# UbiquitousLearning/Mandheling-DSP-Training

Measured on AMD Instinct MI355X. Metric: training images/sec + int8 MFMA TOPS, VGG-11 batch 256, 1/2/4/8 MI355X, higher is better.
Workload: dtype int8; 1 GPU; VGG11 NITI int8 training step (fwd+relu+pool, loss grad, weight grad, input grad, SGD), 3x32x32; global_batch=256, per_gpu_batch=256, parallelism=single GPU, streams=one stream (weight gradient, then input gradient, per layer)

## Files before the change

include/niti_hip.h:

```cpp
#ifndef NITI_HIP_H
#define NITI_HIP_H

#include <stddef.h>
#include <stdint.h>

#ifdef __cplusplus
extern "C" {
#endif

enum niti_error_code {
    NITI_NO_ERROR = 0,
    NITI_OUT_OF_MEMORY = 1,
    NITI_NOT_SUPPORT = 2,
    NITI_COMPUTE_SIZE_ERROR = 3,
    NITI_NO_EXECUTION = 4,
    NITI_INVALID_VALUE = 5,
    NITI_INPUT_DATA_ERROR = 10,
    NITI_CALL_BACK_STOP = 11
};

enum niti_op_type {
    NITI_OP_CONV_INT8 = 700,
    NITI_OP_DECONV_INT8 = 701,
    NITI_OP_RELU_INT8 = 703,
// ... 44 lines not shown
    int kernel_x, kernel_y;
    int stride_x, stride_y;
    int dilate_x, dilate_y;
    int pad_x, pad_y;
    int has_pads;
    int pads[4];
    int pad_mode;
    int input_count, output_count;
    int group;
} niti_conv2d_common;

typedef struct niti_execution* niti_execution_t;

int niti_create_execution(int op_type, const niti_conv2d_common* common, niti_execution_t* out);

int niti_execution_resize(niti_execution_t e, const niti_tensor* inputs, int n_in, const niti_tensor* outputs,
                          int n_out);
int niti_execution_execute(niti_execution_t e, const niti_tensor* inputs, int n_in, const niti_tensor* outputs,
                           int n_out, void* stream);
int niti_execution_status(niti_execution_t e, void* stream);
void niti_destroy_execution(niti_execution_t e);
size_t niti_execution_workspace_bytes(niti_execution_t e);
int niti_tensor_convert(const niti_tensor* src, const niti_tensor* dst, void* stream);

#define NITI_MAX_WORDS 2048
typedef struct niti_geom {
    int n, c_in, h, w, c_out, kh, kw;
    int stride_h, stride_w, pad_t, pad_l, pad_b, pad_r, dilate_h, dilate_w;
    int oh, ow, cip, cop, np;
} niti_geom;

int niti_geom_finalize(niti_geom* g);

int niti_conv_workspace_bytes(const niti_geom* g, int op, size_t* bytes);
int niti_conv_plan_info(const niti_geom* g, int op, size_t ws_bytes, int info[4]);
int niti_conv_plan_set(const niti_geom* g, int op, const int plan[4]);
int niti_matmul_workspace_bytes(int m, int ldc, int k16, size_t* bytes);
int niti_conv_fwd_acc(const niti_geom* g, const int8_t* x_nhwc16, const int8_t* w_ohwi16, int32_t* acc,
                      uint32_t* amax, void* workspace, size_t workspace_bytes, void* stream);
int niti_conv_dgrad_acc(const niti_geom* g, const int8_t* dy_nhwc16, const int8_t* wt_ihwo16, int32_t* acc,
                        uint32_t* amax, void* workspace, size_t workspace_bytes, void* stream);
int niti_conv_fwd_phase1(const niti_geom* g, const int8_t* x_nhwc16, const int8_t* w_ohwi16, int32_t* acc,
                         uint32_t* amax, void* workspace, size_t workspace_bytes, void* stream);
int niti_conv_fwd_phase2(const niti_geom* g, const int8_t* x_nhwc16, const int8_t* w_ohwi16, const int32_t* acc,
                         const uint32_t* amax, const int8_t* exp_in, const int8_t* wscale, int8_t* exp_out, int relu,
                         const int8_t* relu_mask, int8_t* out_nhwc16, size_t workspace_bytes, void* stream);
int niti_conv_dgrad_phase1(const niti_geom* g, const int8_t* dy_nhwc16, const int8_t* wt_ihwo16, int32_t* acc,
                           uint32_t* amax, void* workspace, size_t workspace_bytes, void* stream);
int niti_conv_dgrad_phase2(const niti_geom* g, const int8_t* dy_nhwc16, const int8_t* wt_ihwo16, const int32_t* acc,
                           const uint32_t* amax, const int8_t* exp_in, const int8_t* wscale, int8_t* exp_out,
                           int relu, const int8_t* relu_mask, int8_t* out_nhwc16, size_t workspace_bytes,
                           void* stream);
#define NITI_ROWCONV_STATE_WORDS 1216
uint32_t* niti_rows_spec_slot(uint32_t* state, int dgrad);
int niti_conv_rows_ok(const niti_geom* g);
int niti_nhwc16_to_c32(const int8_t* in_nhwc16, int n, int hw, int cp, int c, int8_t* out_c32, void* stream);
int niti_weights_to_wf(const int8_t* w_ohwi16, int co, int ci, int cip, int transpose, int8_t* out_wf,
                       void* stream);
#define NITI_ROWS_X_NHWC16 0x100
int niti_conv_rows_nhwc_ok(const niti_geom* g, int flags);
int niti_conv_fwd_rows(const niti_geom* g, const int8_t* x_c32, const int8_t* wf, const int8_t* exp_in,
                       const int8_t* wscale, int8_t* exp_out, int relu, int8_t* out_nhwc16, int8_t* pool_out_nhwc16,
                       int8_t* next_c32, int mode, uint32_t* amax, uint32_t* state, uint32_t epoch, uint32_t* err,
                       void* stream);
int niti_conv_dgrad_rows(const niti_geom* g, const int8_t* dy_c32, const int8_t* wft, const int8_t* relu_mask,
                         const int8_t* pool_x, const int8_t* pool_y, int pool_relu, int8_t* dx_nhwc16, int8_t* dx_c32,
                         int8_t* dx_p16, const int8_t* exp_in, const int8_t* wscale, int8_t* exp_out, int mode,
                         uint32_t* amax, uint32_t* state, uint32_t epoch, uint32_t* err, void* stream);
int niti_conv_wgrad_acc(const niti_geom* g, const int8_t* x_nhwc16, const int8_t* dy_nhwc16, int32_t* acc,
                        uint32_t* amax, void* workspace, size_t workspace_bytes, void* stream);
int niti_nhwc16_to_p16(const int8_t* in_nhwc16, int64_t pixels, int cp, int8_t* out_p16, void* stream);
int niti_conv_wgrad_p16_workspace(const niti_geom* g, int splits, size_t* bytes);
void niti_diag_wgrad_stamps(void* buf);
void niti_diag_rowconv_stamps(void* buf);
void niti_diag_rowconv_barrier(uint32_t spin_limit, uint32_t expect_extra);
void niti_diag_rowconv_speculate(int mode);
void niti_diag_gemm_speculate(int bias);
unsigned long long niti_diag_gemm_fused_launches(void);
unsigned long long niti_diag_head_chain_launches(void);
void niti_diag_head_chain(int on);
void niti_diag_p16_jobs_cap(int cap);
int niti_conv_wgrad_p16_acc(const niti_geom* g, const int8_t* x_p16, const int8_t* dy_p16, int32_t* acc,
                            uint32_t* amax, void* workspace, size_t workspace_bytes, int splits, void* stream);
int niti_matmul_acc(int m, int o, int k16, const int8_t* B, int64_t ldb, const int8_t* A, int64_t lda,
                    int32_t* acc, int64_t ldc, uint32_t* amax, void* workspace, size_t workspace_bytes,
                    void* stream);
int niti_absmax_i32(const int32_t* acc, int64_t n, uint32_t* amax, void* stream);
int niti_requant_act(const int32_t* acc, int64_t rows, int ldc, const uint32_t* amax, const int8_t* exp_in,
                     const int8_t* wscale, int8_t* exp_out, int relu, const int8_t* relu_mask, int8_t* out_nhwc16,
                     void* stream);
typedef struct niti_requant_fused {
    const int8_t* exp_in;
    const int8_t* wscale;
    int8_t* exp_out;
    const int8_t* relu_mask;
    int8_t* out_nhwc16;
    int8_t* pool_out;
    const int8_t* pool_x;
    const int8_t* pool_y;
    int8_t* pool_dx;
    int8_t* pool_dx_c32;
    int8_t* out_p16;
    int8_t* pool3_out;
    int8_t* pool3_arg;
    int relu, pool_relu, pool_h, pool_w;
    int zero_cls, zc_h, zc_w;
    int pool3_h, pool3_w, pool3_oh, pool3_ow;
} niti_requant_fused;
int niti_requant_act_fused(const int32_t* acc, int64_t rows, int ldc, const uint32_t* amax,
                           const niti_requant_fused* f, void* stream);
int niti_requant_grad(const int32_t* acc, int64_t n, const uint32_t* amax, int rule, int8_t* g_out,
                      int8_t* w_update, void* stream);
int niti_sgd_update(const int32_t* acc, const uint32_t* amax, int rule, int co, int ci, int kk, int cip, int cop,
                    int8_t* w_ohwi16, int8_t* wt_ihwo16, int8_t* g_out, void* stream);
int niti_sgd_update_wf(const int32_t* acc, const uint32_t* amax, int rule, int co, int ci, int kk, int cip, int cop,
                       int8_t* w_ohwi16, int8_t* wt_ihwo16, int8_t* g_out, int8_t* wf, int8_t* wft, void* stream);
int niti_nhwc16_to_chwn16(const int8_t* in, int n, int hw, int cp, int np, int8_t* out, void* stream);
int niti_ohwi16_to_ihwo16(const int8_t* w, int co, int ci, int kk, int cip, int cop, int8_t* wt, void* stream);
int niti_nchw_to_nhwc16(const int8_t* x, int n, int c, int hw, int cp, int8_t* out, void* stream);
int niti_nchw_to_chwn16(const int8_t* x, int n, int c, int hw, int cp, int np, int8_t* out, void* stream);
int niti_nhwc16_to_nchw(const int8_t* x, int n, int c, int hw, int cp, int8_t* out, void* stream);
int niti_oihw_to_ohwi16(const int8_t* w, int co, int ci, int kk, int cip, int8_t* out, void* stream);
int niti_ohwi16_to_oihw(const int8_t* w, int co, int ci, int kk, int cip, int8_t* out, void* stream);
int niti_residual_add(const int8_t* a, const int8_t* ea, const int8_t* b, const int8_t* eb, int64_t n, int32_t* z,
                      int8_t* ez, uint32_t* amax, void* stream);
int niti_residual_requant(const int8_t* a, const int8_t* ea, const int8_t* b, const int8_t* eb, int64_t n,
                          const uint32_t* amax, int8_t* ez, int8_t* exp_out, int relu, int8_t* out, void* stream);
int niti_residual_requant_relu_grad(const int8_t* a, const int8_t* ea, const int8_t* b, const int8_t* eb, int64_t n,
                                    const uint32_t* amax, int8_t* ez, int8_t* exp_out, const int8_t* relu_mask,
                                    int8_t* out, void* stream);
int niti_sum_pool(const int8_t* x, int n, int hw, int cp, int32_t* acc, uint32_t* amax, void* stream);
int niti_sum_pool_grad(const int8_t* dy, int n, int hw, int cp, int8_t* dx, void* stream);
int niti_im2col(const niti_geom* g, const int8_t* x, int kp, int8_t* xcol, void* stream);
int niti_im2col_nchw(const niti_geom* g, const int8_t* x_nchw, int kp, int8_t* xcol, void* stream);
int niti_maxpool(const int8_t* x, int n, int h, int w, int cp, int k, int s, int p, int8_t* y, int oh, int ow,
                 void* stream);
int niti_maxpool_grad(const int8_t* x, const int8_t* y, const int8_t* dy, int n, int h, int w, int cp, int k,
                      int s, int p, int oh, int ow, int relu, int8_t* dx, void* stream);
int niti_maxpool_grad_ws(const int8_t* x, const int8_t* y, const int8_t* dy, int n, int h, int w, int cp, int k,
                         int s, int p, int oh, int ow, int relu, int8_t* workspace, int8_t* dx, void* stream);
int niti_maxpool_arg(const int8_t* x, int n, int h, int w, int cp, int k, int s, int p, int8_t* y, int oh, int ow,
                     int8_t* arg, void* stream);
int niti_maxpool_grad_arg(const int8_t* x, const int8_t* arg, const int8_t* dy, int n, int h, int w, int cp, int k,
                          int s, int p, int oh, int ow, int relu, const int8_t* pooled, int8_t* dx, void* stream);
int niti_relu_grad(const int8_t* x, const int8_t* dy, int64_t n, int8_t* out, void* stream);
int niti_loss_grad(const int8_t* logits, int batch, int classes, int ld, const int8_t* ascale,
                   const int32_t* labels, int8_t* out, void* stream);
typedef struct niti_eval_totals {
    uint64_t images, top1, topk;
    double loss_sum;
} niti_eval_totals;
int niti_head_metrics(const int8_t* logits, int batch, int classes, int ld, const int8_t* ascale,
                      const int32_t* labels, int topk, int32_t* pred ,
                      double* loss_per_image , niti_eval_totals* totals ,
                      void* workspace, size_t workspace_bytes, void* stream);
int niti_head_metrics_workspace(int batch, size_t* bytes);

int niti_image_stats(const uint8_t* images_nchw, int64_t n, uint64_t* stats, void* stream);
int niti_image_quantize(const uint8_t* images_nchw, int n, int c, int hw, const uint64_t* stats, int64_t count,
                        int8_t* out_nchw, int8_t* ascale, void* stream);
int niti_image_quantize_nhwc16(const uint8_t* images_nchw, int n, int c, int hw, int cp, const uint64_t* stats,
                               int64_t count, int8_t* out_nhwc16, int8_t* ascale, void* stream);

enum niti_arch { NITI_ARCH_LENET = 1, NITI_ARCH_VGG11 = 2, NITI_ARCH_VGG16 = 3, NITI_ARCH_RESNET18 = 4 };
typedef struct niti_model* niti_model_t;

// ... 73 lines not shown
```

mandheling-dsp-training_amd/csrc/niti_capi.hip:

```cpp
#include "../../include/niti_hip.h"
#include <memory>
#include <vector>

#include "niti_internal.hpp"
#include "niti_kernels.hpp"

struct niti_execution {
    niti::Execution* impl = nullptr;
    int op = 0;
    std::vector<void*> stage;
    std::vector<size_t> stage_bytes;
    uint32_t* err_host = nullptr;
    ~niti_execution() {
        delete impl;
        for (void* p : stage)
            if (p) (void)hipFree(p);
        if (err_host) (void)hipHostFree(err_host);
    }
};

namespace {
int code(hipError_t e) {
    if (e == hipSuccess) return NITI_NO_ERROR;
    if (e == hipErrorOutOfMemory) return NITI_OUT_OF_MEMORY;
// ... 367 lines not shown
                         void* ws, size_t ws_bytes, void* stream) {
    if (!g || !x || !w || !acc || !amax) return NITI_INVALID_VALUE;
    niti::ConvGeom r;
    if (!to_geom(g, &r)) return NITI_COMPUTE_SIZE_ERROR;
    return code(niti::conv_fwd_phase1(r, x, w, acc, amax, ws, ws ? ws_bytes : 0, S(stream)));
}

int niti_conv_fwd_phase2(const niti_geom* g, const int8_t* x, const int8_t* w, const int32_t* acc,
                         const uint32_t* amax, const int8_t* exp_in, const int8_t* wscale, int8_t* exp_out, int relu,
                         const int8_t* relu_mask, int8_t* out, size_t ws_bytes, void* stream) {
    if (!g || !x || !w || !acc || !amax || !out) return NITI_INVALID_VALUE;
    niti::ConvGeom r;
    if (!to_geom(g, &r)) return NITI_COMPUTE_SIZE_ERROR;
    return code(niti::conv_fwd_phase2(r, x, w, acc, amax, act_out(exp_in, wscale, exp_out, relu, relu_mask, out),
                                      ws_bytes, S(stream)));
}

int niti_conv_dgrad_phase1(const niti_geom* g, const int8_t* dy, const int8_t* wt, int32_t* acc, uint32_t* amax,
                           void* ws, size_t ws_bytes, void* stream) {
    if (!g || !dy || !wt || !acc || !amax) return NITI_INVALID_VALUE;
    niti::ConvGeom r;
    if (!to_geom(g, &r)) return NITI_COMPUTE_SIZE_ERROR;
    return code(niti::conv_dgrad_phase1(r, dy, wt, acc, amax, ws, ws ? ws_bytes : 0, S(stream)));
}

int niti_conv_dgrad_phase2(const niti_geom* g, const int8_t* dy, const int8_t* wt, const int32_t* acc,
                           const uint32_t* amax, const int8_t* exp_in, const int8_t* wscale, int8_t* exp_out, int relu,
                           const int8_t* relu_mask, int8_t* out, size_t ws_bytes, void* stream) {
    if (!g || !dy || !wt || !acc || !amax || !out) return NITI_INVALID_VALUE;
    niti::ConvGeom r;
    if (!to_geom(g, &r)) return NITI_COMPUTE_SIZE_ERROR;
    return code(niti::conv_dgrad_phase2(r, dy, wt, acc, amax, act_out(exp_in, wscale, exp_out, relu, relu_mask, out),
                                        ws_bytes, S(stream)));
}

int niti_conv_wgrad_acc(const niti_geom* g, const int8_t* x, const int8_t* dy, int32_t* acc, uint32_t* amax,
                        void* ws, size_t ws_bytes, void* stream) {
    if (!g) return NITI_INVALID_VALUE;
    niti::ConvGeom r;
    if (!to_geom(g, &r)) return NITI_COMPUTE_SIZE_ERROR;
    return code(niti::conv_wgrad_acc(r, x, dy, acc, amax, ws, ws_bytes, S(stream)));
}

int niti_nhwc16_to_p16(const int8_t* in, int64_t pixels, int cp, int8_t* out, void* stream) {
    if (!in || !out || pixels <= 0 || pixels % 16 || cp <= 0 || cp % 16) return NITI_INVALID_VALUE;
    return code(niti::nhwc16_to_p16(in, pixels, cp, out, S(stream)));
}

void niti_diag_wgrad_stamps(void* buf) { niti::wgrad_stamps_arm((unsigned long long*)buf); }
void niti_diag_rowconv_stamps(void* buf) { niti::rowconv_stamps_arm((unsigned long long*)buf); }
uint32_t* niti_rows_spec_slot(uint32_t* state, int dgrad) {
    return state ? niti::rowconv_spec_slot(state, dgrad != 0) : nullptr;
}

void niti_diag_rowconv_barrier(uint32_t spin_limit, uint32_t expect_extra) {
    niti::rowconv_barrier_diag(spin_limit, expect_extra);
}
void niti_diag_rowconv_speculate(int mode) { niti::rowconv_speculate(mode); }
void niti_diag_gemm_speculate(int bias) { niti::gemm_speculate_bias(bias); }
unsigned long long niti_diag_gemm_fused_launches(void) { return niti::gemm_fused_launches(); }
unsigned long long niti_diag_head_chain_launches(void) { return niti::head_chain_launches(); }
void niti_diag_head_chain(int on) { niti::head_chain_enable(on); }
void niti_diag_p16_jobs_cap(int cap) { niti::model_p16_jobs_cap(cap); }

int niti_conv_wgrad_p16_workspace(const niti_geom* g, int splits, size_t* bytes) {
    if (!g || !bytes) return NITI_INVALID_VALUE;
    niti::ConvGeom r;
    if (!to_geom(g, &r)) return NITI_COMPUTE_SIZE_ERROR;
    if (!niti::conv_wgrad_p16_ok(r)) return NITI_NOT_SUPPORT;
    *bytes = niti::conv_wgrad_p16_workspace(r, splits);
    return NITI_NO_ERROR;
}

int niti_conv_wgrad_p16_acc(const niti_geom* g, const int8_t* x, const int8_t* dy, int32_t* acc, uint32_t* amax,
                            void* ws, size_t ws_bytes, int splits, void* stream) {
    if (!g || !x || !dy || !acc) return NITI_INVALID_VALUE;
    niti::ConvGeom r;
    if (!to_geom(g, &r)) return NITI_COMPUTE_SIZE_ERROR;
    if (!niti::conv_wgrad_p16_ok(r)) return NITI_NOT_SUPPORT;
    if (splits <= 0) splits = niti::conv_wgrad_p16_splits(r);
    if (ws_bytes < niti::conv_wgrad_p16_workspace(r, splits) || (ws_bytes > 0 && !ws)) return NITI_INVALID_VALUE;
    return code(niti::conv_wgrad_p16(r, x, dy, acc, amax, ws, ws_bytes, splits, S(stream)));
}

int niti_matmul_acc(int m, int o, int k16, const int8_t* B, int64_t ldb, const int8_t* A, int64_t lda, int32_t* acc,
                    int64_t ldc, uint32_t* amax, void* ws, size_t ws_bytes, void* stream) {
    if (k16 % 16 || ldb % 16 || lda % 16 || ldc % 16 || ldc < o) return NITI_INVALID_VALUE;
    return code(niti::matmul_acc(m, o, k16, B, ldb, A, lda, acc, ldc, amax, ws, ws_bytes, S(stream)));
}

int niti_absmax_i32(const int32_t* acc, int64_t n, uint32_t* amax, void* stream) {
    return code(niti::absmax_i32(acc, n, amax, S(stream)));
}

int niti_requant_act(const int32_t* acc, int64_t rows, int ldc, const uint32_t* amax, const int8_t* exp_in,
                     const int8_t* wscale, int8_t* exp_out, int relu, const int8_t* relu_mask, int8_t* out,
                     void* stream) {
    niti::ActRequant r;
    r.acc = acc;
    r.rows = rows;
    r.ldc = ldc;
    r.amax = amax;
    r.exp_in = exp_in;
    r.wscale = wscale;
    r.exp_out = exp_out;
    r.relu = relu;
    r.relu_mask = relu_mask;
    r.out_nhwc16 = out;
    return code(niti::requant_act(r, S(stream)));
}

int niti_requant_act_fused(const int32_t* acc, int64_t rows, int ldc, const uint32_t* amax,
                           const niti_requant_fused* f, void* stream) {
    if (!f || rows < 0) return NITI_INVALID_VALUE;
    niti::ActRequant r;
    r.acc = acc;
    r.rows = rows;
    r.ldc = ldc;
    r.amax = amax;
    r.exp_in = f->exp_in;
    r.wscale = f->wscale;
    r.exp_out = f->exp_out;
    r.relu = f->relu;
    r.relu_mask = f->relu_mask;
    r.out_nhwc16 = f->out_nhwc16;
    r.pool.pool_out = f->pool_out;
    r.pool.x = f->pool_x;
    r.pool.y = f->pool_y;
    r.pool.dx = f->pool_dx;
    r.pool.relu = f->pool_relu;
    r.pool.H = f->pool_h;
    r.pool.W = f->pool_w;
    r.pool.dx_c32 = f->pool_dx_c32;
    r.out_p16 = f->out_p16;
    r.zero_cls = f->zero_cls;
    r.zc_h = f->zc_h;
    r.zc_w = f->zc_w;
    r.pool3.out = f->pool3_out;
    r.pool3.arg = f->pool3_arg;
    r.pool3.H = f->pool3_h;
    r.pool3.W = f->pool3_w;
    r.pool3.OH = f->pool3_oh;
    r.pool3.OW = f->pool3_ow;
    return code(niti::requant_act(r, S(stream)));
}

int niti_requant_grad(const int32_t* acc, int64_t n, const uint32_t* amax, int rule, int8_t* g_out, int8_t* w,
                      void* stream) {
    if (rule != 2 && rule != 3) return NITI_INVALID_VALUE;
    return code(niti::requant_grad(acc, n, amax, rule, g_out, w, S(stream)));
}

int niti_sgd_update(const int32_t* acc, const uint32_t* amax, int rule, int co, int ci, int kk, int cip, int cop,
                    int8_t* w, int8_t* wt, int8_t* g_out, void* stream) {
    if (rule != 2 && rule != 3) return NITI_INVALID_VALUE;
    return code(niti::sgd_update(acc, amax, rule, co, ci, kk, cip, cop, w, wt, g_out, S(stream)));
}
int niti_sgd_update_wf(const int32_t* acc, const uint32_t* amax, int rule, int co, int ci, int kk, int cip, int cop,
                       int8_t* w, int8_t* wt, int8_t* g_out, int8_t* wf, int8_t* wft, void* stream) {
    if (rule != 2 && rule != 3) return NITI_INVALID_VALUE;
    if ((wf || wft) && (kk != 9 || ci % 32 != 0 || co % 32 != 0)) return NITI_NOT_SUPPORT;
    niti::SgdJob j{acc, amax, rule, co, ci, kk, cip, cop, w, wt, g_out};
    j.wf = wf;
    j.wft = wft;
    return code(niti::sgd_update_many(&j, 1, S(stream)));
}
// ... 231 lines not shown
```

mandheling-dsp-training_amd/csrc/niti_kernels.hip:

```cpp
#include <stdlib.h>

#include <map>
#include <atomic>
#include <mutex>
#include <type_traits>
#include <vector>
#include <algorithm>
#include <stdio.h>

#include <hip/hip_ext.h>

#include "niti_device.hpp"
#include "niti_gridbar.hpp"
#include "niti_kernels.hpp"
#include "niti_sgd.hpp"
#include "niti_map.hpp"

namespace niti {


bool ConvGeom::finalize() {
    if (n <= 0 || c_in <= 0 || h <= 0 || w <= 0 || c_out <= 0 || kh <= 0 || kw <= 0) return false;
    if (sh <= 0 || sw <= 0 || dh <= 0 || dw <= 0) return false;
    const int keh = dh * (kh - 1) + 1, kew = dw * (kw - 1) + 1;
// ... 3670 lines not shown
        }
        if (live) {
            const v4i* base = (const v4i*)(J.slab + e);
            const int64_t st4 = J.slab_stride / 4;
            v4i s = {0, 0, 0, 0};
            for (int z0 = 0; z0 < J.splits; z0 += 8) {
                v4i v[8];
#pragma unroll
                for (int q = 0; q < 8; ++q)
                    v[q] = z0 + q < J.splits ? __builtin_nontemporal_load(base + (int64_t)(z0 + q) * st4) : v4i{0, 0, 0, 0};
#pragma unroll
                for (int q = 0; q < 8; ++q) s += v[q];
            }
            *(v4i*)(const_cast<int32_t*>(J.acc) + de) = s;
#pragma unroll
            for (int q = 0; q < 4; ++q) {
                const uint32_t u = uabs32(s[q]);
                m = m > u ? m : u;
            }
        }
    }
    if (cur >= 0) {
        const uint32_t w = wave_max(m);
        if ((threadIdx.x & 63) == 0) publish_max(const_cast<uint32_t*>(jobs.job[cur].amax), w);
    }
}

__global__ void sgd_update_kernel(SgdJobs jobs, int total) {
    __shared__ int8_t T[64][64 + 4];
    struct Tile {
        int j, ci0, co0, k;
    };
    auto locate = [&](int bb) {
        Tile t;
        int b = bb, j = 0;
        while (j + 1 < jobs.n && b >= jobs.start[j + 1]) ++j;
        const SgdJob& J = jobs.job[j];
        b -= jobs.start[j];
        const int tx = (J.cip + 63) / 64, ty = (J.cop + 63) / 64;
        const int k = b / (tx * ty), rem = b - k * tx * ty;
        t.j = j;
        t.ci0 = (rem % tx) * 64;
        t.co0 = (rem / tx) * 64;
        t.k = k;
        return t;
    };
    int bb = blockIdx.x;
    if (bb >= total) return;
    if (!NITI_SGD_PREFETCH) {
        int last_j = -1, bw = 0;
        for (; bb < total; bb += gridDim.x) {
            const Tile t = locate(bb);
            if (t.j != last_j) {
                bw = bitwidth_of(read_max(jobs.job[t.j].amax));
                last_j = t.j;
            }
            if (bb != (int)blockIdx.x) __syncthreads();
            sgd_tile(jobs.job[t.j], bw, t.ci0, t.co0, t.k, T);
        }
        return;
    }
    Tile cur = locate(bb);
    SgdTileIn cin, nin;
    sgd_tile_load(jobs.job[cur.j], cur.ci0, cur.co0, cur.k, cin);
    int last_j = -1, bw = 0;
    for (; bb < total; bb += gridDim.x) {
        const int nb = bb + gridDim.x;
        Tile nxt = cur;
        if (nb < total) {
            nxt = locate(nb);
            sgd_tile_load(jobs.job[nxt.j], nxt.ci0, nxt.co0, nxt.k, nin);
        }
        if (cur.j != last_j) {
            bw = bitwidth_of(read_max(jobs.job[cur.j].amax));
            last_j = cur.j;
        }
        if (bb != (int)blockIdx.x) __syncthreads();
        sgd_tile_finish(jobs.job[cur.j], bw, cur.ci0, cur.co0, cur.k, cin, T);
        cur = nxt;
        cin = nin;
    }
}

hipError_t sgd_update_many(const SgdJob* jobs, int n, hipStream_t st) {
    if (n <= 0) return hipSuccess;
    if (n > SGD_MAX_JOBS) return hipErrorInvalidValue;
    SgdJobs J{};
    J.n = n;
    int total = 0, chunks = 0;
    for (int i = 0; i < n; ++i) {
        J.job[i] = jobs[i];
        J.start[i] = total;
        J.cstart[i] = chunks;
        total += ((jobs[i].cip + 63) / 64) * ((jobs[i].cop + 63) / 64) * jobs[i].kk;
        if (jobs[i].slab != nullptr) {
            if (jobs[i].splits < 1 || jobs[i].slab_stride % 4 != 0 || jobs[i].slab_n % 4 != 0) return hipErrorInvalidValue;
            chunks += (int)((jobs[i].slab_n + 1023) / 1024);
        }
    }
    J.cstart[n] = chunks;
    if (chunks > 0) {
        const int cgrid = chunks < 2048 ? chunks : 2048;
        hipLaunchKernelGGL(sgd_combine_kernel, dim3(cgrid), dim3(256), 0, st, J);
    }
    const int grid = total < 1536 ? total : 1536;
    hipLaunchKernelGGL(sgd_update_kernel, dim3(grid), dim3(256), 0, st, J, total);
    return hipGetLastError();
}

hipError_t sgd_update(const int32_t* acc, const uint32_t* amax, int rule, int co, int ci, int kk, int cip, int cop,
                      int8_t* w, int8_t* wT, int8_t* g_out, hipStream_t st) {
    SgdJob j{acc, amax, rule, co, ci, kk, cip, cop, w, wT, g_out};
    return sgd_update_many(&j, 1, st);
}


__global__ void maxpool_kernel(const int8_t* __restrict__ x, int n, int h, int w, int cp, int k, int s, int p,
                               int8_t* __restrict__ y, int oh, int ow, int8_t* __restrict__ arg) {
    const uint32_t groups = cp / 16;
    const uint32_t total = (uint32_t)n * oh * ow * groups;
    const int kh = k < h ? k : h, kw = k < w ? k : w;
    for (uint32_t t = blockIdx.x * blockDim.x + threadIdx.x; t < total; t += gridDim.x * blockDim.x) {
        uint32_t r = t;
        const int gi = (int)(r % groups);
        r /= groups;
        const int ox = (int)(r % (uint32_t)ow);
        r /= (uint32_t)ow;
        const int oy = (int)(r % (uint32_t)oh);
        const int b = (int)(r / (uint32_t)oh);
        const int sx0 = ox * s - p, sy0 = oy * s - p;
        v16c m, a;
#pragma unroll
        for (int j = 0; j < 16; ++j) {
            m[j] = (signed char)-128;
            a[j] = (signed char)-1;
        }
        for (int yy = max(0, -sy0); yy < min(kh, h - sy0); ++yy)
            for (int xx = max(0, -sx0); xx < min(kw, w - sx0); ++xx) {
                const v16c v = *(const v16c*)(x + (((int64_t)b * h + sy0 + yy) * w + sx0 + xx) * cp + gi * 16);
                const signed char pos = (signed char)(yy * k + xx);
#pragma unroll
                for (int j = 0; j < 16; ++j) {
                    const bool take = a[j] < 0 || v[j] > m[j];
                    m[j] = take ? v[j] : m[j];
                    a[j] = take ? pos : a[j];
                }
            }
        *(v16c*)(y + (int64_t)t * 16) = m;
        if (arg != nullptr && (kh < k || kw < k)) {
#pragma unroll
            for (int j = 0; j < 16; ++j) a[j] = (signed char)-1;
            for (int yy = max(0, -sy0); yy < min(k, h - sy0); ++yy)
                for (int xx = max(0, -sx0); xx < min(k, w - sx0); ++xx) {
                    const v16c v = *(const v16c*)(x + (((int64_t)b * h + sy0 + yy) * w + sx0 + xx) * cp + gi * 16);
                    const signed char pos = (signed char)(yy * k + xx);
#pragma unroll
                    for (int j = 0; j < 16; ++j) a[j] = (a[j] < 0 && v[j] >= m[j]) ? pos : a[j];
                }
        }
        if (arg != nullptr) *(v16c*)(arg + (int64_t)t * 16) = a;
    }
}

hipError_t maxpool_nhwc16(const int8_t* x, int n, int h, int w, int cp, int k, int s, int p, int8_t* y, int oh, int ow,
                          hipStream_t st, int8_t* arg) {
    const int64_t total = (int64_t)n * oh * ow * (cp / 16);
// ... 641 lines not shown
```

mandheling-dsp-training_amd/csrc/niti_kernels.hpp:

```cpp
#pragma once

#include <hip/hip_runtime.h>
#include <stdint.h>
#include <stdlib.h>

#include "../../include/niti_hip.h"

namespace niti {

inline int round_up(int x, int m) { return (x + m - 1) / m * m; }

constexpr int MAX_SLOTS = 64;
constexpr int MAX_SLOT_STRIDE = 32;
constexpr int MAX_WORDS = MAX_SLOTS * MAX_SLOT_STRIDE;
constexpr size_t MAX_BYTES = MAX_WORDS * sizeof(uint32_t);

struct ConvGeom {
    int n, c_in, h, w;
    int c_out, kh, kw;
    int sh, sw, pt, pl, pb, pr, dh, dw;
    int oh, ow;
    int cip, cop, np;
    bool finalize();
};

enum GradRule { RULE_WGRAD_BW2 = 2, RULE_MATMUL_BW3 = 3 };

size_t conv_fwd_workspace(const ConvGeom& g);
size_t conv_dgrad_workspace(const ConvGeom& g);
size_t conv_wgrad_workspace(const ConvGeom& g);
size_t matmul_workspace(int M, int ldc, int k16);

enum PlanOp { PLAN_FWD = 0, PLAN_DGRAD = 1, PLAN_WGRAD = 2, PLAN_MATMUL = 3 };
struct PlanKey {
    int op, M, N, K;
    bool operator<(const PlanKey& o) const {
        if (op != o.op) return op < o.op;
        if (M != o.M) return M < o.M;
        if (N != o.N) return N < o.N;
        return K < o.K;
    }
};
struct PlanChoice {
    int bm = 128, bn = 128, splits = 1, strat = 0;
};
constexpr int PLAN_TAPS_TILE = 32;
constexpr int PLAN_P16_TILE = 16;
bool plan_override_lookup(const PlanKey& k, PlanChoice* c);
bool conv_wgrad_taps_ok(const ConvGeom& g);
PlanKey conv_plan_key(int op, const ConvGeom& g);
PlanChoice conv_plan_query(int op, const ConvGeom& g, bool recompute_ok, size_t ws_bytes);
int conv_plan_k_step(int op, const ConvGeom& g);
void plan_override_set(const PlanKey& k, const PlanChoice& c);
void plan_override_clear(const PlanKey& k);
void plan_override_clear_all();
unsigned plan_override_epoch();
PlanChoice plan_query(const PlanKey& k, int k_step, bool recompute_ok, size_t ws_bytes);
size_t plan_slab_bytes(int M, int N, int splits);
struct PlanChoice;
size_t conv_wgrad_slab_bytes(const ConvGeom& g, const PlanChoice& c);
hipError_t conv_fwd_acc(const ConvGeom& g, const int8_t* x_nhwc16, const int8_t* w_ohwi16, int32_t* acc,
                        uint32_t* amax, void* ws, size_t ws_bytes, hipStream_t st);
hipError_t conv_dgrad_acc(const ConvGeom& g, const int8_t* dy_nhwc16, const int8_t* wt_ihwo16, int32_t* acc,
                          uint32_t* amax, void* ws, size_t ws_bytes, hipStream_t st);
void probe_span_arm(unsigned long long* slot);
constexpr int SPAN_MAX_BLOCKS = 4096;
void probe_events_arm(hipEvent_t begin, hipEvent_t end);
struct SgdJob;
hipError_t conv_wgrad_acc(const ConvGeom& g, const int8_t* x_nhwc16, const int8_t* dy_nhwc16, int32_t* acc,
                          uint32_t* amax, void* ws, size_t ws_bytes, hipStream_t st, hipEvent_t after_gemm = nullptr,
                          SgdJob* defer = nullptr);
hipError_t splitk_reduce_linear(const int32_t* slab, int splits, int64_t n, int64_t stride, int32_t* C,
                                uint32_t* amax, hipStream_t st);
hipError_t residual_fused(const int8_t* a, const int8_t* ea, const int8_t* b, const int8_t* eb, int64_t n, int8_t* ez,
                          int8_t* exp_out, int relu, int8_t* out, uint32_t* bar, uint32_t epoch, uint32_t* err,
                          hipStream_t st, const int8_t* relu_mask = nullptr);
int resident_wgs(const void* f, int threads = 256);
hipError_t residual_add(const int8_t* a, const int8_t* ea, const int8_t* b, const int8_t* eb, int64_t n,
                        int32_t* z, int8_t* ez, uint32_t* amax, hipStream_t st);
constexpr int RES_SPEC_SLOT_WORDS = 32;
hipError_t residual_requant(const int8_t* a, const int8_t* ea, const int8_t* b, const int8_t* eb, int64_t n,
                            const uint32_t* amax, int8_t* ez, int8_t* exp_out, int relu, int8_t* out, hipStream_t st,
                            const int8_t* relu_mask = nullptr, int spec = 0, uint32_t* slot = nullptr);
hipError_t sum_pool(const int8_t* x, int n, int hw, int cp, int32_t* acc, uint32_t* amax, hipStream_t st);
hipError_t sum_pool_grad(const int8_t* dy, int n, int hw, int cp, int8_t* dx, hipStream_t st,
                         const int8_t* relu_mask = nullptr);
hipError_t im2col_small(const ConvGeom& g, const int8_t* x, int kp, int8_t* xcol, hipStream_t st, bool nchw = false);
hipError_t nhwc16_to_p16(const int8_t* in, int64_t pixels, int cp, int8_t* out, hipStream_t st);
struct P16Conv {
    const int8_t* in = nullptr;
    int64_t pixels = 0;
    int cp = 0;
    int8_t* out = nullptr;
};
constexpr int P16_MAX_JOBS = 16;
hipError_t nhwc16_to_p16_many(const P16Conv* jobs, int n, hipStream_t st);
hipError_t loss_grad_p16(const int8_t* logits, int batch, int classes, int ld, const int8_t* ascale,
                         const int32_t* labels, int8_t* out, const P16Conv* jobs, int n, hipStream_t st);
bool conv_wgrad_p16_ok(const ConvGeom& g);
void wgrad_stamps_arm(unsigned long long* buf);
int conv_wgrad_p16_splits(const ConvGeom& g);
size_t conv_wgrad_p16_workspace(const ConvGeom& g, int splits);
struct SgdJob;
hipError_t conv_wgrad_p16(const ConvGeom& g, const int8_t* x_p16, const int8_t* dy_p16, int32_t* acc,
                          uint32_t* amax, void* ws, size_t ws_bytes, int splits, hipStream_t st,
                          hipEvent_t ev_b = nullptr, hipEvent_t ev_e = nullptr, unsigned long long* span = nullptr,
                          SgdJob* defer = nullptr);
hipError_t matmul_acc(int M, int O, int k16, const int8_t* B, int64_t ldb, const int8_t* A, int64_t lda,
                      int32_t* acc, int64_t ldc, uint32_t* amax, void* ws, size_t ws_bytes, hipStream_t st);

struct PoolFuse {
    int8_t* pool_out = nullptr;
    const int8_t* x = nullptr;
    const int8_t* y = nullptr;
    int8_t* dx = nullptr;
    int relu = 0;
    int H = 0, W = 0;
    int8_t* dx_c32 = nullptr;
};
struct Pool3 {
    int8_t* out = nullptr;
    int8_t* arg = nullptr;
    int H = 0, W = 0, OH = 0, OW = 0;
};
struct ActOut {
    int8_t* out = nullptr;
    int relu = 0;
    const int8_t* relu_mask = nullptr;
    const int8_t* exp_in = nullptr;
    const int8_t* wscale = nullptr;
    int8_t* exp_out = nullptr;
    PoolFuse pool;
    int8_t* out_p16 = nullptr;
    int zero_cls = 0, zc_h = 0, zc_w = 0;
    Pool3 pool3;
};
bool conv_fwd_phase2_separate(const ConvGeom& g, size_t ws_bytes);
bool conv0_ok(const ConvGeom& g);
hipError_t conv0_fwd(const ConvGeom& g, const int8_t* xcol, const int8_t* w, uint32_t* amax, const ActOut& o,
                     int pass, hipStream_t st,
                     int8_t* pool_c32 = nullptr, int8_t* out_c32 = nullptr, int8_t* pool_code = nullptr);
bool conv_dgrad_phase2_separate(const ConvGeom& g, size_t ws_bytes);
constexpr int GEMM_SPEC_SLOT_WORDS = 32;
constexpr int GEMM_SPEC_ALT_PAIRS = 8;
inline bool tune_spec() {
    static const bool on = getenv("NITI_TUNE_SPEC") && atoi(getenv("NITI_TUNE_SPEC")) == 1;
    return on;
}
bool conv_fwd_spec_ok(const ConvGeom& g);
bool conv_dgrad_spec_ok(const ConvGeom& g);
void gemm_speculate_bias(int bias);
size_t conv_fwd_spec_alt_bytes(const ConvGeom& g);
size_t conv_dgrad_spec_alt_bytes(const ConvGeom& g);
hipError_t conv_fwd_spec(const ConvGeom& g, const int8_t* x, const int8_t* w, uint32_t* amax, const ActOut& o,
                         uint32_t* slot, int pass, hipStream_t st, int8_t* alt = nullptr);
hipError_t conv_dgrad_spec(const ConvGeom& g, const int8_t* dy, const int8_t* wt, uint32_t* amax, const ActOut& o,
                           uint32_t* slot, int pass, hipStream_t st, int8_t* alt = nullptr);
struct FusedBar {
    uint32_t* bar = nullptr;
    uint32_t epoch = 0;
    uint32_t* err = nullptr;
    uint32_t spin_limit = 0;
};
unsigned long long gemm_fused_launches();
hipError_t conv_fwd_fused(const ConvGeom& g, const int8_t* x, const int8_t* w, const ActOut& o, const FusedBar& fb,
                          hipStream_t st);
hipError_t conv_dgrad_fused(const ConvGeom& g, const int8_t* dy, const int8_t* wt, const ActOut& o, const FusedBar& fb,
                            hipStream_t st);
hipError_t conv_fwd_phase1(const ConvGeom& g, const int8_t* x, const int8_t* w, int32_t* acc, uint32_t* amax,
                           void* ws, size_t ws_bytes, hipStream_t st);
hipError_t conv_fwd_phase2(const ConvGeom& g, const int8_t* x, const int8_t* w, const int32_t* acc,
                           const uint32_t* amax, const ActOut& o, size_t ws_bytes, hipStream_t st);
hipError_t conv_dgrad_phase1(const ConvGeom& g, const int8_t* dy, const int8_t* wt, int32_t* acc, uint32_t* amax,
                             void* ws, size_t ws_bytes, hipStream_t st, const int8_t* subw = nullptr);
hipError_t conv_dgrad_phase2(const ConvGeom& g, const int8_t* dy, const int8_t* wt, const int32_t* acc,
                             const uint32_t* amax, const ActOut& o, size_t ws_bytes, hipStream_t st,
                             const int8_t* subw = nullptr);
bool conv_dgrad_subpix_ok(const ConvGeom& g);
size_t conv_dgrad_subpix_bytes(const ConvGeom& g);
hipError_t conv_dgrad_subpix_weights(const ConvGeom& g, const int8_t* wt, int8_t* out, hipStream_t st);

struct RowConvOut {
    int8_t* out = nullptr;
    int8_t* pool_out = nullptr;
    int8_t* next = nullptr;
    const int8_t* exp_in = nullptr;
    const int8_t* wscale = nullptr;
    int8_t* exp_out = nullptr;
    int relu = 0;
    const int8_t* relu_mask = nullptr;
    const int8_t* pool_x = nullptr;
    const int8_t* pool_y = nullptr;
    int8_t* pool_dx = nullptr;
    int8_t* pool_dx_next = nullptr;
    int pool_relu = 0;
    const int8_t* pool_code = nullptr;
    int8_t* pool_code_out = nullptr;
    int pool_dx_nhwc = 1;
    int8_t* p16 = nullptr;
    int32_t* acc_store = nullptr;
    int dgrad_slot = 0;
    int x_nhwc = 0;
};
size_t rowconv_acc_bytes(const ConvGeom& g, bool dg);
bool rowconv_nhwc_ok(const ConvGeom& g);
bool rowconv_nhwc_pref(const ConvGeom& g);
constexpr int ROWCONV_BAR_WORDS = 2 * 19 * 32;
static_assert(ROWCONV_BAR_WORDS == NITI_ROWCONV_STATE_WORDS, "header constant");
bool rowconv_ok(const ConvGeom& g);
bool rowconv_seg(const ConvGeom& g);
bool rowconv_dgrad_geom(const ConvGeom& layer, ConvGeom* d);
bool rowconv_p16_ok(const ConvGeom& d, bool pool);
bool rowconv_fused_ok(const ConvGeom& g, bool dg = false);
int rowconv_units(const ConvGeom& g, bool dg = false);
size_t rowconv_wf_bytes(int co, int ci);
hipError_t nhwc16_to_c32(const int8_t* in, int n, int hw, int cp, int c, int8_t* out, hipStream_t st);
hipError_t c32_to_nhwc16(const int8_t* in, int n, int hw, int cp, int c, int8_t* out, hipStream_t st);
hipError_t weights_to_wf(const int8_t* w_ohwi16, int co, int ci, int cip, bool transpose, int8_t* out,
                         hipStream_t st);
constexpr int RC_SPEC_A = 3, RC_SPEC_B = 4;
bool rowconv_spec2_on();
void rowconv_stamps_arm(unsigned long long* buf);
void rowconv_barrier_diag(uint32_t spin_limit, uint32_t expect_extra);
void rowconv_speculate(int mode);
uint32_t* rowconv_spec_slot(uint32_t* bar, bool dg);
void model_p16_jobs_cap(int cap);
hipError_t rowconv_fwd(const ConvGeom& g, const int8_t* x_c32, const int8_t* wf, const RowConvOut& o, int mode,
                       uint32_t* amax, uint32_t* bar, uint32_t epoch, uint32_t* err, hipStream_t st);
struct HeadChain {
    const int8_t* x = nullptr;
    int xld = 0;
    const int8_t* w = nullptr;
    const int8_t* wT = nullptr;
    int n = 0, K = 0, c_out = 0, cop = 0, relu = 0;
    const int8_t* exp_in = nullptr;
    const int8_t* wscale = nullptr;
    int8_t* exp_out = nullptr;
    int8_t* logits = nullptr;
    const int32_t* labels = nullptr;
    int8_t* dy = nullptr;
    int32_t* dw = nullptr;
    uint32_t* dw_amax = nullptr;
    const int8_t* code = nullptr;
    int8_t* pool_dx = nullptr;
    int8_t* pool_dx_c32 = nullptr;
    int8_t* p16 = nullptr;
    int G = 0;
    int stamps = 0;
};
bool head_chain_ok(int n, int K, int c_out, int cop);
hipError_t head_chain(const HeadChain& h, hipStream_t st);
unsigned long long head_chain_launches();
bool head_chain_enabled();
void head_chain_enable(int on);
bool rowconv_fc_ok(int n, int K, int rows, bool fused);
hipError_t head_wgrad(int n, int c_out, int cip, const int8_t* x, int xld, const int8_t* dy, int dld, int32_t* dw,
                      uint32_t* amax, hipStream_t st);
hipError_t rowconv_fc(int n, int K, int rows, const int8_t* x, int xld, const int8_t* w, int wld,
                      const RowConvOut& o, int mode, uint32_t* amax, uint32_t* bar, uint32_t epoch, uint32_t* err,
                      hipStream_t st);

hipError_t absmax_i32(const int32_t* a, int64_t n, uint32_t* amax, hipStream_t st);
struct AbsmaxJob {
    const int32_t* a;
    int64_t n;
    uint32_t* amax;
    uint32_t b0;
};
constexpr int ABSMAX_MAX_JOBS = 24;
struct AbsmaxJobs {
    AbsmaxJob j[ABSMAX_MAX_JOBS];
    int n;
};
hipError_t absmax_many(const AbsmaxJob* jobs, int n, hipStream_t st);

struct ActRequant {
    const int32_t* acc = nullptr;
    int64_t rows = 0;
    int ldc = 0;
    const uint32_t* amax = nullptr;
    const int8_t* exp_in = nullptr;
    const int8_t* wscale = nullptr;
    int8_t* exp_out = nullptr;
    int relu = 0;
    const int8_t* relu_mask = nullptr;
    int8_t* out_nhwc16 = nullptr;
    int8_t* out_c4 = nullptr;
    int c_real = 0, n = 0, hw = 0;
    PoolFuse pool;
    int8_t* out_p16 = nullptr;
    int zero_cls = 0, zc_h = 0, zc_w = 0;
    Pool3 pool3;
};
hipError_t requant_act(const ActRequant& r, hipStream_t st);
bool requant_p16_ok(const ActRequant& r);

hipError_t requant_grad(const int32_t* acc, int64_t n, const uint32_t* amax, int rule, int8_t* g_out,
                        int8_t* w_update, hipStream_t st);

struct SgdJob {
    const int32_t* acc;
    const uint32_t* amax;
    int rule, co, ci, kk, cip, cop;
    int8_t* w;
    int8_t* wT;
    int8_t* g_out;
    int8_t* wf = nullptr;
    int8_t* wft = nullptr;
    int8_t* subw = nullptr;
    int sub_kw = 0, sub_kh = 0, sub_pt = 0, sub_pl = 0;
    const int32_t* slab = nullptr;
    int splits = 0;
    int64_t slab_stride = 0, slab_n = 0;
    int slab_map = 0;
    int tb_tiles_ci = 0, tb_cip4 = 0, tb_ld4 = 0;
    uint32_t tb_m = 0, tb_s = 0;
};
constexpr int SGD_MAX_JOBS = 24;
struct SgdJobs {
    SgdJob job[SGD_MAX_JOBS];
    int start[SGD_MAX_JOBS];
    int cstart[SGD_MAX_JOBS + 1];
    int n;
};
hipError_t sgd_update_many(const SgdJob* jobs, int n, hipStream_t st);
bool conv_wgrad_fc_sgd_ok(const ConvGeom& g);
hipError_t conv_wgrad_fc_sgd(const ConvGeom& g, const int8_t* x, const int8_t* dy, uint32_t* amax, const SgdJob& j,
                             int pass, hipStream_t st);
hipError_t grad_exponent(const uint32_t* amax, int rule, int8_t* out, hipStream_t st);
hipError_t sgd_update(const int32_t* acc, const uint32_t* amax, int rule, int co, int ci, int kk, int cip, int cop,
                      int8_t* w, int8_t* wT, int8_t* g_out, hipStream_t st);

hipError_t maxpool_nhwc16(const int8_t* x, int n, int h, int w, int cp, int k, int s, int p, int8_t* y,
                          int oh, int ow, hipStream_t st, int8_t* arg = nullptr);
hipError_t maxpool_relu_grad_nhwc16(const int8_t* x, const int8_t* y, const int8_t* dy, int n, int h,
                                    int w, int cp, int k, int s, int p, int oh, int ow, int relu,
                                    int8_t* dx, hipStream_t st);
hipError_t relu_grad_nhwc16(const int8_t* x, const int8_t* dy, int64_t n, int8_t* out, hipStream_t st);
hipError_t maxpool_relu_grad_ws(const int8_t* x, const int8_t* y, const int8_t* dy, int n, int h, int w, int cp, int k,
                                int s, int p, int oh, int ow, int relu, int8_t* ws, int8_t* dx, hipStream_t st);
hipError_t maxpool_relu_grad_arg(const int8_t* x, const int8_t* arg, const int8_t* dy, int n, int h, int w, int cp,
                                 int k, int s, int p, int oh, int ow, int relu, int8_t* dx, hipStream_t st,
                                 const int8_t* pooled = nullptr);
hipError_t loss_grad(const int8_t* logits, int batch, int classes, int ld, const int8_t* ascale,
                     const int32_t* labels, int8_t* out, hipStream_t st);
size_t head_metrics_workspace(int batch);
hipError_t head_metrics(const int8_t* logits, int batch, int classes, int ld, const int8_t* ascale,
                        const int32_t* labels, int topk, int32_t* pred, double* loss_per_image,
                        niti_eval_totals* totals, void* workspace, size_t workspace_bytes, hipStream_t st);

hipError_t batch_gather(const uint8_t* data, const int32_t* labels, int64_t count, int c, int h, int w,
                        const int32_t* index, const int32_t* xform, int n, uint8_t* out, int32_t* labels_out,
                        hipStream_t st);
bool resize_size_ok(int in, int out);
hipError_t batch_gather_resize(const uint8_t* data, const int32_t* labels, int64_t count, int c, int h, int w,
                               const int32_t* index, const int32_t* xform, const int32_t* window, int n, int oh,
                               int ow, uint8_t* out, int32_t* labels_out, hipStream_t st);

hipError_t image_stats(const uint8_t* img, int64_t n, unsigned long long* stats, hipStream_t st);
hipError_t image_quantize(const uint8_t* img, int n, int c, int hw, int cp, const unsigned long long* stats,
                          int64_t count, int8_t* out, int8_t* ascale, bool nhwc16, hipStream_t st);
constexpr int IMAGE_STATS_SLOTS = 256;
hipError_t image_stats_slots(const uint8_t* img, int64_t n, unsigned long long* slots, int* nslots, hipStream_t st,
                             void* zero = nullptr, size_t zero_bytes = 0);
hipError_t stats_finalize(const unsigned long long* slots, int nslots, unsigned long long* stats, hipStream_t st);
bool input_im2col_ok(int c, int kh, int kw);
struct Conv0Range {
    const int8_t* w = nullptr;
    int co = 0, cop = 0;
    uint32_t* amax = nullptr;
};
hipError_t input_im2col(const void* in, bool quant, int n, int c, int h, int w, int kh, int kw, int pt, int pl,
                        const unsigned long long* slots, int nslots, int64_t count, int8_t* x_nchw, int8_t* xcol,
                        int8_t* ascale, hipStream_t st, const Conv0Range& r0 = Conv0Range{});

hipError_t nhwc16_to_chwn16(const int8_t* in, int n, int hw, int cp, int np, int8_t* out, hipStream_t st);
hipError_t ohwi16_to_ihwo16(const int8_t* w, int co, int ci, int kk, int cip, int cop, int8_t* wt,
                            hipStream_t st);
hipError_t c4_to_nhwc16(const int8_t* x_c4, int n, int c, int hw, int cp, int8_t* out, hipStream_t st);
hipError_t nchw_to_nhwc16(const int8_t* x, int n, int c, int hw, int cp, int8_t* out, hipStream_t st);
hipError_t nchw_to_chwn16(const int8_t* x, int n, int c, int hw, int cp, int np, int8_t* out,
                          hipStream_t st);
hipError_t c4_to_chwn16(const int8_t* x_c4, int n, int c, int hw, int cp, int np, int8_t* out,
                        hipStream_t st);
hipError_t nhwc16_to_nchw(const int8_t* x, int n, int c, int hw, int cp, int8_t* out, hipStream_t st);
hipError_t oihw_to_ohwi16(const int8_t* w, int co, int ci, int kk, int cip, int8_t* out, hipStream_t st,
                          bool reverse_taps = false);
hipError_t oihw_to_ihwo16(const int8_t* w, int co, int ci, int kk, int cop, int8_t* out, hipStream_t st);
hipError_t ohwi16_to_oihw(const int8_t* w, int co, int ci, int kk, int cip, int8_t* out, hipStream_t st);
hipError_t pad_rows(const int8_t* in, int rows, int cols, int ld, int8_t* out, hipStream_t st);
hipError_t transpose_i32(const int32_t* in, int rows, int cols, int ld, int32_t* out, hipStream_t st);

}
```

mandheling-dsp-training_amd/csrc/niti_model.hip:

```cpp
#include <stdlib.h>
#include <string.h>

#include <algorithm>
#include <memory>
#include <vector>

#include "../../include/niti_hip.h"
#include "niti_map.hpp"
#include "niti_step_driver.hpp"

namespace niti {

namespace {
extern int g_p16_jobs_cap;
}
void model_p16_jobs_cap(int cap) { g_p16_jobs_cap = cap <= 0 ? P16_MAX_JOBS : cap; }

namespace {

template <int C, int KH, int KW>
struct Im2Col32 {
    const int8_t* x;
    int cip, h, w, oh, ow, c, kh, kw, sh, sw, pt, pl;
    int8_t* out;
    __device__ void operator()(int64_t p) const {
        typedef signed char v16c_t __attribute__((ext_vector_type(16)));
        const int64_t img = p / ((int64_t)oh * ow);
        const int r = (int)(p - img * oh * ow);
        const int oy = r / ow, ox = r - (r / ow) * ow;
        const int8_t* base = x + img * h * w * cip;
        if constexpr (C > 0) {
            v16c_t v[2] = {v16c_t{}, v16c_t{}};
#pragma unroll
            for (int ky = 0; ky < KH; ++ky)
#pragma unroll
                for (int kx = 0; kx < KW; ++kx) {
                    const int iy = oy * sh + ky - pt, ix = ox * sw + kx - pl;
                    const bool ok = iy >= 0 && iy < h && ix >= 0 && ix < w;
                    const v16c_t px = ok ? *(const v16c_t*)(base + ((int64_t)iy * w + ix) * cip) : v16c_t{};
#pragma unroll
                    for (int ch = 0; ch < C; ++ch) {
                        const int k = (ky * KW + kx) * C + ch;
                        v[k >> 4][k & 15] = px[ch];
                    }
                }
            *(v16c_t*)(out + p * 32) = v[0];
            *(v16c_t*)(out + p * 32 + 16) = v[1];
        } else {
            int k = 0;
            for (int ky = 0; ky < kh; ++ky)
                for (int kx = 0; kx < kw; ++kx) {
                    const int iy = oy * sh + ky - pt, ix = ox * sw + kx - pl;
                    const bool ok = iy >= 0 && iy < h && ix >= 0 && ix < w;
                    for (int ch = 0; ch < c; ++ch, ++k)
                        out[p * 32 + k] = ok ? base[((int64_t)iy * w + ix) * cip + ch] : (int8_t)0;
                }
            for (; k < 32; ++k) out[p * 32 + k] = 0;
        }
    }
};

int g_p16_jobs_cap = P16_MAX_JOBS;

static hipError_t im2col32(const ConvGeom& o, const int8_t* x16, int8_t* out, hipStream_t st) {
    const int64_t px = (int64_t)o.n * o.oh * o.ow;
    const int cip = round_up(o.c_in, 16);
    if (o.c_in == 3 && o.kh == 3 && o.kw == 3)
        return launch_map(px, Im2Col32<3, 3, 3>{x16, cip, o.h, o.w, o.oh, o.ow, 3, 3, 3, o.sh, o.sw, o.pt, o.pl, out}, st);
    if (o.c_in == 1 && o.kh == 5 && o.kw == 5)
        return launch_map(px, Im2Col32<1, 5, 5>{x16, cip, o.h, o.w, o.oh, o.ow, 1, 5, 5, o.sh, o.sw, o.pt, o.pl, out}, st);
    return launch_map(px, Im2Col32<0, 0, 0>{x16, cip, o.h, o.w, o.oh, o.ow, o.c_in, o.kh, o.kw, o.sh, o.sw, o.pt, o.pl,
                                            out},
                      st);
}

struct FlattenFwd {
    const int8_t* in;
    int hw, c, cp, ldo;
    int8_t* out;
    __device__ void operator()(int64_t i) const {
        const int64_t b = i / ldo;
        const int j = (int)(i - b * ldo);
        const int ch = j / hw, p = j - ch * hw;
        out[i] = ch < c ? in[(b * hw + p) * cp + ch] : (int8_t)0;
    }
};
struct FlattenBwd {
    const int8_t* dout;
    int hw, c, cp, ldo;
    int8_t* din;
    __device__ void operator()(int64_t i) const {
        const int ch = (int)(i % cp);
        const int64_t r = i / cp;
        const int p = (int)(r % hw);
        const int64_t b = r / hw;
        din[i] = ch < c ? dout[b * ldo + ch * hw + p] : (int8_t)0;
    }
};

}

struct Layer {
    ConvGeom g{};
    int relu = 0, pool = 0, flatten = 0;
    int ph = 0, pw = 0;
    int8_t wscale = 0;
    int8_t* w = nullptr;
    int8_t* ws_dev = nullptr;
    int8_t* wT = nullptr;
    int8_t* r = nullptr;
    int8_t* p = nullptr;
    int8_t* pc = nullptr;
    bool r_written = false;
    int8_t* flat = nullptr;
    int8_t* dy = nullptr;
    int8_t* dtmp = nullptr;
    int8_t* dflat = nullptr;
    int32_t* dwacc = nullptr;
    int32_t* slab16 = nullptr;
    size_t slab16_bytes = 0;
    int32_t* wslab = nullptr;
    size_t wslab_bytes = 0;
    SgdJob defer{};
    bool fc_sgd = false;
    int8_t* g8 = nullptr;
    int8_t* exp = nullptr;
    const int8_t* in = nullptr;
    int col = 0;
    ConvGeom og{};
    int8_t* xcol = nullptr;
    int rc = 0;
    int8_t* xc32 = nullptr;
    int8_t* wf = nullptr;
    uint32_t* bar = nullptr;
    uint32_t epoch = 0;
    int rcd = 0;
    ConvGeom dg{};
    uint32_t* gspec = nullptr;
    int8_t* wft = nullptr;
    int8_t* dyc32 = nullptr;
    int64_t w_elems() const { return (int64_t)g.c_out * g.kh * g.kw * g.cip; }
    int64_t macs() const { return (int64_t)og.n * og.oh * og.ow * og.c_out * og.c_in * og.kh * og.kw; }
};

struct Model final : StepDriver {
// ... 125 lines not shown
    struct Key {
        const void* x = nullptr;
        const void* labels = nullptr;
        int exp_in = 0, pl = -1, pp = -1;
        bool operator==(const Key& o) const {
            return x == o.x && labels == o.labels && exp_in == o.exp_in && pl == o.pl && pp == o.pp;
        }
    } key;
    hipError_t cap_err = hipSuccess;
    void drop_graph() override {
        for (auto e : segs) (void)hipGraphExecDestroy(e);
        segs.clear();
    }
    void seg_cut(hipStream_t st) {
        hipGraph_t g = nullptr;
        hipError_t e = hipStreamEndCapture(st, &g);
        hipGraphExec_t ex = nullptr;
        if (e == hipSuccess) e = hipGraphInstantiate(&ex, g, nullptr, nullptr, 0);
        if (g) (void)hipGraphDestroy(g);
        if (e == hipSuccess) segs.push_back(ex);
        if (cap_err == hipSuccess) cap_err = e;
        e = hipStreamBeginCapture(st, hipStreamCaptureModeThreadLocal);
        if (cap_err == hipSuccess) cap_err = e;
    }
    unsigned long long* span = nullptr;
    int span_cap = 0, span_count = 0;
    void arm_kernel_events(int layer, int phase) {
        if (layer != probe_layer || phase != probe_phase || probe_paused || tuning || capturing || probe_count >= (int)ev0.size())
            return;
        probe_events_arm(ev0[probe_count], ev1[probe_count]);
        ++probe_count;
    }
    void arm_span(int layer, int phase) {
        if (layer != probe_layer || phase != probe_phase || probe_paused || tuning || capturing || span == nullptr ||
            span_count >= span_cap)
            return;
        probe_span_arm(span + 2 * SPAN_MAX_BLOCKS * span_count++);
    }
    void probe(int layer, int phase, bool begin, hipStream_t st) {
        if (layer != probe_layer || phase != probe_phase || tuning) return;
        if (capturing) {
            seg_cut(st);
            return;
        }
        if (probe_paused) return;
        if (probe_count >= (int)ev0.size()) return;
        if (begin) {
            (void)hipEventRecord(ev0[probe_count], st);
        } else {
            (void)hipEventRecord(ev1[probe_count], st);
            ++probe_count;
        }
    }
    hipEvent_t probe_end_event(int layer, int phase) {
        if (layer != probe_layer || phase != probe_phase || probe_paused || capturing || tuning || probe_count >= (int)ev0.size())
            return nullptr;
        return ev1[probe_count++];
    }
    void clear_probe() override {
        StepDriver::clear_probe();
        if (span) (void)hipFree(span);
        span = nullptr;
        span_cap = span_count = 0;
    }
    int probe_alloc(int phase, int max_launches) override;
    int probe_read_span(double* total_ms, int* count) override;

    int build(int arch_, int batch_, int in_hw = 0);
    int fwd_layer(int i, hipStream_t st);
    int wgrad_layer(int i, hipStream_t st);
    int dgrad_layer(int i, hipStream_t st);
    bool head_chain_on() const {
        const int h = (int)L.size() - 1;
        if (!head_chain_enabled() || h < 1 || dp() || tuning || probe_layer == h) return false;
        const Layer& l = L[h];
        return head_layer(h) && head_dgrad_ok(h) && L[h - 1].pool && pool_code_layer(h - 1) &&
               head_chain_ok(batch, l.g.cip, l.g.c_out, l.g.cop) && L[h - 1].g.cop == l.g.cip && l.g.kh * l.g.kw == 1;
    }
    bool skip_dy16(int i, const int8_t* next, const int8_t* p16) const {
        static const bool keep = getenv("NITI_DY16") != nullptr && getenv("NITI_DY16")[0] == '1';
        return !keep && i - 1 >= 1 && next != nullptr && p16 != nullptr && wgrad_p16_splits(i - 1) > 0;
    }
    int autotune(hipStream_t st, int reps) override;
    size_t ws_bytes_for(int op) const { return op == PLAN_WGRAD ? slab_w_bytes : slab_bytes; }
    bool ensure_wslab(int i) const {
        const Layer& l = L[i];
        const PlanChoice c = conv_plan_query(PLAN_WGRAD, l.g, false, slab_w_bytes);
        if (c.strat != 2 || c.splits < 2 || c.bm == PLAN_P16_TILE) return false;
        return l.wslab_bytes >= conv_wgrad_slab_bytes(l.g, c);
    }
    unsigned wslab_epoch = 0;
    int size_wslabs() {
        if (wslab_epoch == plan_override_epoch()) return NITI_NO_ERROR;
        bool synced = false;
        for (Layer& l : L) {
            const PlanChoice c = conv_plan_query(PLAN_WGRAD, l.g, false, slab_w_bytes);
            if (c.strat != 2 || c.splits < 2 || c.bm == PLAN_P16_TILE) continue;
            const size_t need = conv_wgrad_slab_bytes(l.g, c);
            if (l.wslab_bytes >= need) continue;
            if (!synced && hipDeviceSynchronize() != hipSuccess) return NITI_NO_EXECUTION;
            synced = true;
            void* p = ws.replace(l.wslab, need);
            l.wslab = (int32_t*)p;
            l.wslab_bytes = p ? need : 0;
            if (!p) return NITI_OUT_OF_MEMORY;
        }
        wslab_epoch = plan_override_epoch();
        return NITI_NO_ERROR;
    }
    int ensure_streams() {
        if (side) return NITI_NO_ERROR;
        if (hipStreamCreateWithFlags(&side, hipStreamNonBlocking) != hipSuccess) return NITI_NO_EXECUTION;
        constexpr unsigned kFlags = hipEventDisableTiming | hipEventReleaseToDevice;
        if (hipEventCreateWithFlags(&ev_side, kFlags) != hipSuccess) return NITI_NO_EXECUTION;
        ev_dy.resize(L.size());
        for (auto& e : ev_dy)
            if (hipEventCreateWithFlags(&e, kFlags) != hipSuccess) return NITI_NO_EXECUTION;
        return NITI_NO_ERROR;
    }
    int run(const int8_t* x_nchw, int exp_in, const uint8_t* images, const int32_t* labels, hipStream_t st);
    int step(const int8_t* x_nchw, int exp_in, const uint8_t* images, const int32_t* labels, hipStream_t st) override;
    int forward(const int8_t* x_nchw, int exp_in, const uint8_t* images, bool skip_head, hipStream_t st);
    int backward(bool head_chain, const int32_t* labels, SgdJob* jobs, hipStream_t st);
    int eval(const int8_t* x_nchw, int exp_in, const uint8_t* images, const int32_t* labels, hipStream_t st) override;
    int copy_weights_from(StepDriver& src, hipStream_t st) override;
    int run_phase(int layer, int phase, hipStream_t st) override;
    int plan_info(int layer, int phase, int info[4]) override;
    int plan_set(int layer, int phase, const int plan[4]) override;
    int set_rowconv(bool enable) override;
    void set_overlap(bool enable) override { overlap = enable; }
    bool layer_ok(int layer) const { return layer >= 0 && layer < (int)L.size(); }
    int num_layers() const override { return (int)L.size(); }
    int layer_info(int layer, int info[12]) const override;
    int set_weight(int layer, const int8_t* w_oihw_host, int wscale) override;
    int get_weight(int layer, int8_t* w_oihw_host) override;
    int get_tap(int layer, int which, int8_t* host, size_t bytes, hipStream_t st) override;
    int get_logits(int8_t* host, int* exp_out, hipStream_t st) override;
    void logits_view(const int8_t** logits, int* classes, int* ld, const int8_t** exp) const override {
        const Layer& t = L.back();
        *logits = t.r;
        *classes = t.g.c_out;
        *ld = t.g.cop;
        *exp = t.exp;
    }
    int get_input(int8_t* host, int* ascale, hipStream_t st) override;
    int64_t step_macs() const override;
    int spec_stats(uint32_t* out, int max_layers) override;
    int spec_state(int layer, uint32_t** bar) override {
        if (!layer_ok(layer)) return NITI_INVALID_VALUE;
        *bar = L[layer].bar;
        return NITI_NO_ERROR;
    }
    ~Model() override {
        clear_probe();
        drop_graph();
        if (cst) (void)hipStreamSynchronize(cst);
        for (auto e : ev_dy) (void)hipEventDestroy(e);
        if (ev_side) (void)hipEventDestroy(ev_side);
        if (side) (void)hipStreamDestroy(side);
    }
};

static void add_conv(Model& m, int ci, int co, int k, int pad, int h, int relu, int pool, int flatten = 0) {
    Layer l;
    l.g.n = m.batch;
    l.g.c_in = ci;
    l.g.h = l.g.w = h;
    l.g.c_out = co;
    l.g.kh = l.g.kw = k;
    l.g.sh = l.g.sw = 1;
    l.g.pt = l.g.pl = l.g.pb = l.g.pr = pad;
    l.g.dh = l.g.dw = 1;
    l.g.finalize();
    l.og = l.g;
    l.relu = relu;
    l.pool = pool;
    l.flatten = flatten;
    if (pool) {
        l.ph = (l.g.oh - 2) / 2 + 1;
        l.pw = (l.g.ow - 2) / 2 + 1;
    }
    m.L.push_back(l);
}

int Model::build(int arch_, int batch_, int in_hw) {
    arch = arch_;
    batch = batch_;
    if (arch == NITI_ARCH_LENET) {
        in_c = 1;
        in_h = in_w = 28;
// ... 102 lines not shown
        l.gspec = (uint32_t*)ws.alloc(2 * GEMM_SPEC_SLOT_WORDS * 4);
        if (!l.w || !l.ws_dev || !l.wT || !l.r || !l.dy || !l.dwacc || !l.g8 || !l.exp || !l.gspec)
            return NITI_OUT_OF_MEMORY;
        if (hipMemset(l.gspec, 0, 2 * GEMM_SPEC_SLOT_WORDS * 4) != hipSuccess) return NITI_NO_EXECUTION;
        if (hipMemset(l.w, 0, l.w_elems()) != hipSuccess) return NITI_NO_EXECUTION;
        if (hipMemset(l.ws_dev, 0, 16) != hipSuccess) return NITI_NO_EXECUTION;
        acc_elems = std::max(acc_elems, out_px * g.cop);
        acc_elems = std::max(acc_elems, (size_t)n * g.h * g.w * g.cip);
        slab_bytes = std::max(slab_bytes, conv_fwd_workspace(g));
        slab_bytes = std::max(slab_bytes, conv_dgrad_workspace(g));
        slab_w_bytes = std::max(slab_w_bytes, conv_wgrad_workspace(g));
        l.bar = (uint32_t*)ws.alloc(ROWCONV_BAR_WORDS * 4);
        if (!l.bar || hipMemset(l.bar, 0, ROWCONV_BAR_WORDS * 4) != hipSuccess) return NITI_OUT_OF_MEMORY;
        if (!l.col && rowconv_ok(g)) {
            l.rc = 1;
            l.wf = (int8_t*)ws.alloc(rowconv_wf_bytes(g.c_out, g.c_in));
            l.xc32 = (int8_t*)ws.alloc((size_t)n * round_up(g.c_in, 32) * g.h * g.w);
            if (!l.wf || !l.xc32) return NITI_OUT_OF_MEMORY;
            if (hipMemset(l.wf, 0, rowconv_wf_bytes(g.c_out, g.c_in)) != hipSuccess)
                return NITI_NO_EXECUTION;
            rc_acc_size = std::max(rc_acc_size, rowconv_acc_bytes(g, false));
            const Layer* pv = i > 0 ? &L[i - 1] : nullptr;
            const bool pv_ok = pv != nullptr && !pv->flatten && pv->g.cop == g.cip &&
                               (pv->pool ? (pv->ph == g.h && pv->pw == g.w && pv->g.oh == 2 * g.h && pv->g.ow == 2 * g.w)
                                         : (pv->g.oh == g.h && pv->g.ow == g.w));
            if (pv_ok && rowconv_dgrad_geom(g, &l.dg)) {
                l.rcd = 1;
                rc_acc_size = std::max(rc_acc_size, rowconv_acc_bytes(l.dg, true));
                l.wft = (int8_t*)ws.alloc(rowconv_wf_bytes(g.c_in, g.c_out));
                l.dyc32 = (int8_t*)ws.alloc(out_px * round_up(g.c_out, 32));
                if (!l.wft || !l.dyc32) return NITI_OUT_OF_MEMORY;
                if (hipMemset(l.wft, 0, rowconv_wf_bytes(g.c_in, g.c_out)) != hipSuccess) return NITI_NO_EXECUTION;
            }
        }
        if (conv_wgrad_p16_ok(g)) {
            slab_w_bytes = std::max(slab_w_bytes, conv_wgrad_p16_workspace(g, 8));
            xp16[i] = (int8_t*)ws.alloc((size_t)n * g.h * g.w * g.cip);
            l.slab16_bytes = conv_wgrad_p16_workspace(g, 8);
            l.slab16 = l.slab16_bytes ? (int32_t*)ws.alloc(l.slab16_bytes) : nullptr;
            if (l.slab16_bytes && !l.slab16) return NITI_OUT_OF_MEMORY;
            dp16[i] = (int8_t*)ws.alloc(out_px * g.cop);
            if (!xp16[i] || !dp16[i]) return NITI_OUT_OF_MEMORY;
        }
        if (i == 0) {
            l.in = l.col ? l.xcol : x0;
        } else {
            const Layer& pr = L[i - 1];
            l.in = pr.flatten ? pr.flat : (pr.pool ? pr.p : pr.r);
        }
    }
    acc = (int32_t*)ws.alloc(acc_elems * 4);
    qstats = (unsigned long long*)ws.alloc(64);
    qslots = (unsigned long long*)ws.alloc((size_t)IMAGE_STATS_SLOTS * 4 * sizeof(unsigned long long));
    x0n = (int8_t*)ws.alloc((size_t)n * in_c * in_h * in_w);
    if (!qstats || !qslots || !x0n) return NITI_OUT_OF_MEMORY;
    if (slab_bytes) {
        slab = ws.alloc(slab_bytes);
        if (!slab) return NITI_OUT_OF_MEMORY;
    }
    if (slab_w_bytes) {
        slab_w = ws.alloc(slab_w_bytes);
        if (!slab_w) return NITI_OUT_OF_MEMORY;
    }
    if (rc_acc_size) {
        rc_acc = (int32_t*)ws.alloc(rc_acc_size);
        if (!rc_acc) return NITI_OUT_OF_MEMORY;
    }
    for (int i = 0; i < nl; ++i) {
        const Layer& l = L[i];
        if (!(l.col && conv0_ok(l.g)) && !l.rc) gspec_alt_bytes = std::max(gspec_alt_bytes, conv_fwd_spec_alt_bytes(l.g));
        if (i > 0 && !l.rcd) gspec_alt_bytes = std::max(gspec_alt_bytes, conv_dgrad_spec_alt_bytes(l.g));
    }
    if (gspec_alt_bytes && !(gspec_alt = (int8_t*)ws.alloc(gspec_alt_bytes))) return NITI_OUT_OF_MEMORY;
    amax_bytes = (size_t)3 * nl * MAX_BYTES;
    amax = (uint32_t*)ws.alloc(amax_bytes);
    if (const int rc = alloc_eval()) return rc;
    if (!x0 || !exp0 || !acc || !amax) return NITI_OUT_OF_MEMORY;
    for (int i = 0; i < nl; ++i) grads.push_back(GradSlot{L[i].dwacc, L[i].w_elems(), rng(i, 2)});
    if (hipMemset(x0, 0, (size_t)n * in_h * in_w * round_up(in_c, 16)) != hipSuccess) return NITI_NO_EXECUTION;
    return hipDeviceSynchronize() == hipSuccess ? NITI_NO_ERROR : NITI_NO_EXECUTION;
}

int Model::step(const int8_t* x_nchw, int exp_in, const uint8_t* images, const int32_t* labels, hipStream_t st) {
    if (!use_graph || coll != nullptr) return run(x_nchw, exp_in, images, labels, st);
    Key k;
    k.x = x_nchw ? (const void*)x_nchw : (const void*)images;
    k.labels = labels;
    k.exp_in = exp_in;
    k.pl = probe_layer;
    k.pp = probe_phase;
    if (segs.empty() || !(k == key)) {
        drop_graph();
        if (const int rc = ensure_graph_stream()) return rc;
        DTRY(hipStreamBeginCapture(gstream, hipStreamCaptureModeThreadLocal));
        capturing = true;
        cap_err = hipSuccess;
        const int rc = run(x_nchw, exp_in, images, labels, gstream);
        hipGraph_t g = nullptr;
        hipError_t e = hipStreamEndCapture(gstream, &g);
        capturing = false;
        hipGraphExec_t ex = nullptr;
        if (e == hipSuccess && rc == NITI_NO_ERROR) e = hipGraphInstantiate(&ex, g, nullptr, nullptr, 0);
        if (g) (void)hipGraphDestroy(g);
        if (e == hipSuccess && rc == NITI_NO_ERROR) segs.push_back(ex);
        if (rc != NITI_NO_ERROR || e != hipSuccess || cap_err != hipSuccess || (segs.size() != 1 && segs.size() != 3)) {
            drop_graph();
            use_graph = false;
            (void)hipGetLastError();
            return run(x_nchw, exp_in, images, labels, st);
        }
        key = k;
    }
    DTRY(hipEventRecord(gin, st));
    DTRY(hipStreamWaitEvent(gstream, gin, 0));
    const bool probing = segs.size() == 3 && !probe_paused && probe_count < (int)ev0.size();
    for (size_t j = 0; j < segs.size(); ++j) {
        if (probing && j == 1) DTRY(hipEventRecord(ev0[probe_count], gstream));
        if (probing && j == 2) DTRY(hipEventRecord(ev1[probe_count++], gstream));
        DTRY(hipGraphLaunch(segs[j], gstream));
    }
    DTRY(hipEventRecord(gout, gstream));
    DTRY(hipStreamWaitEvent(st, gout, 0));
    return NITI_NO_ERROR;
}

int Model::fwd_layer(int i, hipStream_t st) {
    const int n = batch;
    const bool dp = this->dp();
    Layer& l = L[i];
    const ConvGeom& g = l.g;
    probe(i, 0, true, st);
    l.r_written = true;
    if (l.col && conv0_ok(g) && !l.flatten) {
        ActOut o;
        const bool code = pool_code_layer(i);
        l.r_written = keep_grads || !code;
        o.out = l.r_written ? l.r : nullptr;
        o.relu = l.relu;
        o.exp_in = exp0;
        o.wscale = l.ws_dev;
        o.exp_out = l.exp;
        o.pool.pool_out = l.pool ? l.p : nullptr;
        const bool next_c32 = i + 1 < (int)L.size() && rowconv_layer(i + 1) && !rowconv_nhwc_pref(L[i + 1].g);
        if (!conv0_ranged) DTRY(conv0_fwd(g, l.in, l.w, rng(i, 0), o, 0, st));
        conv0_ranged = false;
        if (dp && exact) DTRY(coll->allreduce(rng(i, 0), MAX_WORDS, COLL_MAX_U32, st));
        DTRY(conv0_fwd(g, l.in, l.w, rng(i, 0), o, 1, st, next_c32 && l.pool ? L[i + 1].xc32 : nullptr,
                       next_c32 && !l.pool ? L[i + 1].xc32 : nullptr, code ? l.pc : nullptr));
        if (next_c32) xc32_valid[i + 1] = 1;
        probe(i, 0, false, st);
        return NITI_NO_ERROR;
    }
    if (head_layer(i)) {
        RowConvOut o;
        o.out = l.r;
        o.exp_in = i == 0 ? exp0 : L[i - 1].exp;
        o.wscale = l.ws_dev;
        o.exp_out = l.exp;
        o.relu = l.relu;
        const int K = g.c_in, rows = g.c_out;
        if (!dp && !capturing && rowconv_fc_ok(n, K, rows, true)) {
            DTRY(rowconv_fc(n, K, rows, l.in, g.cip, l.w, g.cip, o, 0, rng(i, 0), l.bar, ++l.epoch, rc_err, st));
        } else if (rowconv_spec2_on()) {
            DTRY(rowconv_fc(n, K, rows, l.in, g.cip, l.w, g.cip, o, RC_SPEC_A, rng(i, 0), l.bar, 0, nullptr, st));
            if (dp && exact) DTRY(coll->allreduce(rng(i, 0), MAX_WORDS, COLL_MAX_U32, st));
            DTRY(rowconv_fc(n, K, rows, l.in, g.cip, l.w, g.cip, o, RC_SPEC_B, rng(i, 0), l.bar, 0, nullptr, st));
// ... 288 lines not shown
                        FlattenBwd{pv.dflat, pv.ph * pv.pw, pg.c_out, pg.cop, ld, pv.dtmp}, st));
        DTRY(maxpool_relu_grad_nhwc16(pv.r, pv.p, pv.dtmp, n, pg.oh, pg.ow, pg.cop, 2, 2, 0, pv.ph, pv.pw, pv.relu,
                                      pv.dy, st));
    } else if (pv.pool && !fuse) {
        DTRY(maxpool_relu_grad_nhwc16(pv.r, pv.p, pv.dtmp, n, pg.oh, pg.ow, pg.cop, 2, 2, 0, pv.ph, pv.pw, pv.relu,
                                      pv.dy, st));
    }
    if (o.out_p16 != nullptr) dp16_valid[i - 1] = 1;
    dyc32_valid[i - 1] = fuse && o.pool.dx_c32 != nullptr ? 1 : 0;
    return NITI_NO_ERROR;
}

int Model::autotune(hipStream_t st, int reps) {
    if (reps < 1) reps = 5;
    const int nl = (int)L.size();
    if (!ensure_slab(size_t(96) << 20, false) || !ensure_slab(size_t(96) << 20, true)) return NITI_OUT_OF_MEMORY;
    drop_graph();
    TuneTimer timer;
    if (const int rc = timer.init(st, reps)) return rc;
    tuning = true;
    int rc = NITI_NO_ERROR;
    if (hipMemsetAsync(amax, 0, amax_bytes, st) != hipSuccess) rc = NITI_NO_EXECUTION;
    const bool log = getenv("NITI_DIAG_TUNE_LOG") != nullptr;
    for (int i = 0; i < nl && rc == NITI_NO_ERROR; ++i) {
        for (int op : {PLAN_FWD, PLAN_WGRAD, PLAN_DGRAD}) {
            if (op == PLAN_DGRAD && i == 0) continue;
            if (op == PLAN_FWD && rowconv_layer(i)) continue;
            if (op == PLAN_DGRAD && rowconv_dgrad_layer(i)) continue;
            if ((op == PLAN_FWD && head_layer(i)) || (op == PLAN_DGRAD && head_dgrad_ok(i))) continue;
            if (op == PLAN_WGRAD && head_layer(i) && L[i].g.c_out <= 32 && L[i].g.cip % 32 == 0) continue;
            const ConvGeom& g = L[i].g;
            const PlanKey key = conv_plan_key(op, g);
            auto time_op = [&](float* us) {
                return timer.time(
                    [&] { return op == PLAN_FWD ? fwd_layer(i, st) : op == PLAN_WGRAD ? wgrad_layer(i, st) : dgrad_layer(i, st); },
                    us);
            };
            auto note = [&](const PlanChoice& c, float us) {
                if (log) fprintf(stderr, "tune layer %d op %d plan (%d,%d,%d,%d) %.2f us\n", i, op, c.bm, c.bn, c.splits, c.strat, us);
            };
            plan_override_clear(key);
            const size_t wsb = ws_bytes_for(op);
            PlanChoice best = conv_plan_query(op, g, op != PLAN_WGRAD, wsb);
            if (op == PLAN_WGRAD && wgrad_p16_splits(i) > 0) {
                best.bm = best.bn = PLAN_P16_TILE;
                best.splits = wgrad_p16_splits(i);
                best.strat = best.splits > 1 ? 2 : 0;
            }
            invalidate_xp16();
            if (op == PLAN_WGRAD && conv_wgrad_p16_ok(g)) {
                if (nhwc16_to_p16(L[i].in, (int64_t)g.n * g.h * g.w, g.cip, xp16[i], st) != hipSuccess) {
                    rc = NITI_NO_EXECUTION;
                    break;
                }
                xp16_valid[i] = 1;
            }
            float best_us = 0.f;
            rc = time_op(&best_us);
            note(best, best_us);
            if (op == PLAN_WGRAD && conv_wgrad_p16_ok(g)) {
                for (int sp : {1, 2, 4, 8}) {
                    if (rc != NITI_NO_ERROR) break;
                    if (conv_wgrad_p16_workspace(g, sp) > slab_w_bytes) continue;
                    PlanChoice cand;
                    cand.bm = cand.bn = PLAN_P16_TILE;
                    cand.splits = sp;
                    cand.strat = sp > 1 ? 2 : 0;
                    plan_override_set(key, cand);
                    float us = 0.f;
                    rc = time_op(&us);
                    note(cand, us);
                    if (rc == NITI_NO_ERROR && us < best_us) {
                        best_us = us;
                        best = cand;
                    }
                }
            }
            if (rc == NITI_NO_ERROR) rc = tune_gemm_tiles(op, g, wsb, time_op, note, &best, &best_us);
            plan_override_set(key, best);
            invalidate_xp16();
            if (rc != NITI_NO_ERROR) break;
        }
    }
    invalidate_xp16();
    tuning = false;
    if (hipStreamSynchronize(st) != hipSuccess) rc = NITI_NO_EXECUTION;
    return rc;
}

int Model::run(const int8_t* x_nchw, int exp_in, const uint8_t* images, const int32_t* labels, hipStream_t st) {
    const int nl = (int)L.size();
    const bool dp = this->dp();
    SgdJob jobs[SGD_MAX_JOBS];
    if (nl > SGD_MAX_JOBS) return NITI_NOT_SUPPORT;
    struct InStep {
        bool& f;
        explicit InStep(bool& x) : f(x) { f = true; }
        ~InStep() { f = false; }
    } in_step_guard(in_step);
    for (auto& l : L) l.defer = SgdJob{};
    if (dp) {
        const int rc = ensure_comm_stream();
        if (rc != NITI_NO_ERROR) return rc;
    }
    if (!dp && !capturing && !tuning) {
        const int rc = size_wslabs();
        if (rc != NITI_NO_ERROR) return rc;
    }
    std::fill(dyc32_valid.begin(), dyc32_valid.end(), 0);
    const bool hc = head_chain_on();
    {
        const int rc = forward(x_nchw, exp_in, images, hc, st);
        if (rc != NITI_NO_ERROR) return rc;
    }
    return backward(hc, labels, jobs, st);
}

int Model::forward(const int8_t* x_nchw, int exp_in, const uint8_t* images, bool skip_head, hipStream_t st) {
    const int n = batch;
    const int nl = (int)L.size();
    const bool dp = this->dp();
    invalidate_xp16();
    std::fill(xc32_valid.begin(), xc32_valid.end(), 0);
    auto fill = [&](void* p, int v, size_t bytes) {
        return eval_pass || capturing ? fill_kernel(p, v, bytes, st) : hipMemsetAsync(p, v, bytes, st);
    };
    if (x_nchw != nullptr || amax_bytes % 16 != 0) DTRY(fill(amax, 0, amax_bytes));
    const ConvGeom& o0 = L[0].og;
    const bool fused_in = L[0].col && input_im2col_ok(o0.c_in, o0.kh, o0.kw) && o0.sh == 1 && o0.sw == 1;
    x0_nchw_valid = fused_in;
    Conv0Range r0;
    if (fused_in && conv0_ok(L[0].g) && !L[0].flatten && L[0].g.cop <= 64) {
        r0.w = L[0].w;
        r0.co = L[0].g.c_out;
        r0.cop = L[0].g.cop;
        r0.amax = rng(0, 0);
    }
    conv0_ranged = r0.w != nullptr;
    if (x_nchw != nullptr) {
        DTRY(fill(exp0, exp_in, 1));
        if (fused_in)
            DTRY(input_im2col(x_nchw, false, n, in_c, in_h, in_w, o0.kh, o0.kw, o0.pt, o0.pl, nullptr, 0, 0, x0n,
                              L[0].xcol, nullptr, st, r0));
        else
            DTRY(nchw_to_nhwc16(x_nchw, n, in_c, in_h * in_w, round_up(in_c, 16), x0, st));
    } else {
        const int64_t px = (int64_t)n * in_c * in_h * in_w;
        int ns = 0;
        DTRY(image_stats_slots(images, px, qslots, &ns, st, amax_bytes % 16 == 0 ? amax : nullptr,
                               amax_bytes % 16 == 0 ? amax_bytes : 0));
        const unsigned long long* slots = qslots;
        if ((dp && exact) || !fused_in) {
            DTRY(stats_finalize(qslots, ns, qstats, st));
            slots = qstats;
            ns = 1;
        }
        if (dp && exact) {
            DTRY(coll->allreduce(qstats, 2, COLL_SUM_U64, st));
            DTRY(coll->allreduce(qstats + 2, 2, COLL_MAX_U64, st));
        }
        const int64_t count = dp && exact ? px * world : px;
        if (fused_in)
            DTRY(input_im2col(images, true, n, in_c, in_h, in_w, o0.kh, o0.kw, o0.pt, o0.pl, slots, ns, count, x0n,
                              L[0].xcol, exp0, st, r0));
        else
            DTRY(image_quantize(images, n, in_c, in_h * in_w, round_up(in_c, 16), qstats, count, x0, exp0, true, st));
    }
    if (L[0].col && !fused_in) DTRY(im2col32(L[0].og, x0, L[0].xcol, st));
    for (int i = 0; i < nl - (skip_head ? 1 : 0); ++i) {
        const int rc = fwd_layer(i, st);
        if (rc != NITI_NO_ERROR) return rc;
    }
    return NITI_NO_ERROR;
}

int Model::backward(bool hc, const int32_t* labels, SgdJob* jobs, hipStream_t st) {
    const int n = batch;
    const int nl = (int)L.size();
    const bool dp = this->dp();
    const bool ov = overlap && !capturing && !(dp && shared_comm);
    bool p16_done = false;
    {
        Layer& t = L[nl - 1];
        P16Conv jobs[P16_MAX_JOBS];
        int nj = 0;
        if (hc) {
            const bool with_jobs = !ov && p16_input_jobs(jobs, &nj);
            if (!with_jobs) nj = 0;
            Layer& pv = L[nl - 2];
            HeadChain h;
            h.x = t.in;
            h.xld = t.g.cip;
            h.w = t.w;
            h.wT = t.wT;
            h.n = n;
            h.K = t.g.cip;
            h.c_out = t.g.c_out;
            h.cop = t.g.cop;
            h.relu = t.relu;
            h.exp_in = pv.exp;
            h.wscale = t.ws_dev;
            h.exp_out = t.exp;
            h.logits = t.r;
            h.labels = labels;
            h.dy = t.dy;
            h.dw = t.dwacc;
            h.dw_amax = rng(nl - 1, 2);
            h.code = pv.pc;
            int8_t* next = rowconv_dgrad_layer(nl - 2) && !rowconv_nhwc_pref(pv.dg) ? pv.dyc32 : nullptr;
            h.p16 = fuse_dp16 && wgrad_p16_splits(nl - 2) > 0 ? dp16[nl - 2] : nullptr;
            h.pool_dx = skip_dy16(nl - 1, next, h.p16) ? nullptr : pv.dy;
            h.pool_dx_c32 = next;
            DTRY(head_chain(h, st));
            if (with_jobs && nj > 0) {
                DTRY(nhwc16_to_p16_many(jobs, nj, st));
                for (int j = 0; j < nl; ++j)
                    if (wgrad_p16_splits(j)) xp16_valid[j] = 1;
                p16_done = true;
            }
            t.r_written = true;
            dy16_valid[nl - 1] = 1;
            dy16_valid[nl - 2] = h.pool_dx != nullptr;
            dp16_valid[nl - 2] = h.p16 != nullptr ? 1 : 0;
            dyc32_valid[nl - 2] = next != nullptr ? 1 : 0;
        } else if (!ov && p16_input_jobs(jobs, &nj) && nj > 0) {
            DTRY(loss_grad_p16(t.r, n, t.g.c_out, t.g.cop, t.exp, labels, t.dy, jobs, nj, st));
            for (int j = 0; j < nl; ++j)
                if (wgrad_p16_splits(j)) xp16_valid[j] = 1;
            p16_done = true;
        } else {
            DTRY(loss_grad(t.r, n, t.g.c_out, t.g.cop, t.exp, labels, t.dy, st));
        }
        dp16_valid[nl - 1] = 0;
    }
    if (ov) {
        const int rc = ensure_streams();
        if (rc != NITI_NO_ERROR) return rc;
    }
    hipStream_t wst = ov ? side : st;
    for (int i = nl - 1; i >= 0; --i) {
        if (ov) {
            DTRY(hipEventRecord(ev_dy[i], st));
            DTRY(hipStreamWaitEvent(side, ev_dy[i], 0));
        }
        if (i == nl - 1 && !p16_done) {
            const int rc = convert_p16_inputs(wst);
            if (rc != NITI_NO_ERROR) return rc;
        }
        Layer& l = L[i];
        const ConvGeom& g = l.g;
        const bool in_chain = hc && i == nl - 1;
        int rc = in_chain ? NITI_NO_ERROR : wgrad_layer(i, wst);
        if (rc == NITI_NO_ERROR && dp && closes_bucket[i]) rc = sum_bucket(i, wst);
        if (rc == NITI_NO_ERROR && i > 0 && !in_chain) rc = dgrad_layer(i, st);
        if (rc != NITI_NO_ERROR) return rc;
        jobs[i] = SgdJob{l.dwacc, rng(i, 2), RULE_WGRAD_BW2, g.c_out, g.c_in, g.kh * g.kw, g.cip, g.cop, l.w,
                         i > 0 && !rowconv_dgrad_layer(i) ? l.wT : nullptr, keep_grads ? l.g8 : nullptr};
        jobs[i].wf = l.rc ? l.wf : nullptr;
        jobs[i].wft = l.rcd ? l.wft : nullptr;
        if (l.defer.slab != nullptr) {
            jobs[i].slab = l.defer.slab;
            jobs[i].splits = l.defer.splits;
            jobs[i].slab_stride = l.defer.slab_stride;
            jobs[i].slab_n = l.defer.slab_n;
            jobs[i].slab_map = l.defer.slab_map;
            jobs[i].tb_tiles_ci = l.defer.tb_tiles_ci;
            jobs[i].tb_cip4 = l.defer.tb_cip4;
            jobs[i].tb_ld4 = l.defer.tb_ld4;
            jobs[i].tb_m = l.defer.tb_m;
            jobs[i].tb_s = l.defer.tb_s;
        }
    }
    if (dp) {
        DTRY(hipEventRecord(ev_grads, cst));
        DTRY(hipStreamWaitEvent(st, ev_grads, 0));
    } else if (ov) {
        DTRY(hipEventRecord(ev_side, side));
        DTRY(hipStreamWaitEvent(st, ev_side, 0));
    }
    SgdJob many[SGD_MAX_JOBS];
    int n_many = 0;
    for (int i = 0; i < nl; ++i)
        if (!L[i].fc_sgd) many[n_many++] = jobs[i];
    DTRY(sgd_update_many(many, n_many, st));
    for (int i = 0; i < nl; ++i)
        if (L[i].fc_sgd) DTRY(conv_wgrad_fc_sgd(L[i].g, L[i].in, L[i].dy, rng(i, 2), jobs[i], 1, st));
    g8_written = keep_grads;
    return NITI_NO_ERROR;
}

int Model::eval(const int8_t* x_nchw, int exp_in, const uint8_t* images, const int32_t* labels, hipStream_t st) {
    const bool paused = probe_paused;
    probe_paused = true;
    eval_pass = true;
    const int rc = forward(x_nchw, exp_in, images, false, st);
    eval_pass = false;
    probe_paused = paused;
    if (rc != NITI_NO_ERROR) return rc;
    const Layer& t = L.back();
    DTRY(head_metrics(t.r, batch, t.g.c_out, t.g.cop, t.exp, labels, std::min(ev_topk, t.g.c_out), ev_pred, nullptr,
                      ev_totals, ev_ws, ev_ws_bytes, st));
    return NITI_NO_ERROR;
}

int Model::copy_weights_from(StepDriver& other, hipStream_t st) {
    Model* sp = dynamic_cast<Model*>(&other);
    if (sp == nullptr) return NITI_INVALID_VALUE;
    Model& src = *sp;
    if (src.arch != arch || src.in_h != in_h || src.in_w != in_w || src.in_c != in_c || src.L.size() != L.size())
        return NITI_INVALID_VALUE;
    for (size_t i = 0; i < L.size(); ++i) {
        const ConvGeom &a = L[i].g, &b = src.L[i].g;
        if (a.c_in != b.c_in || a.c_out != b.c_out || a.kh != b.kh || a.kw != b.kw || a.cip != b.cip || a.cop != b.cop ||
            L[i].col != src.L[i].col)
            return NITI_INVALID_VALUE;
    }
    if (&src == this) return NITI_NO_ERROR;
    for (size_t i = 0; i < L.size(); ++i) {
        Layer& l = L[i];
        const Layer& s = src.L[i];
        const ConvGeom& g = l.g;
        DTRY(copy_kernel(l.w, s.w, (size_t)l.w_elems(), st));
        DTRY(copy_kernel(l.ws_dev, s.ws_dev, 1, st));
        l.wscale = s.wscale;
        if (!l.rcd)
            DTRY(ohwi16_to_ihwo16(l.w, g.c_out, g.c_in, g.kh * g.kw, g.cip, g.cop, l.wT, st));
    }
    int rc = refresh_wt(st);
    if (rc == NITI_NO_ERROR) rc = refresh_wf(st);
    return rc;
}

int Model::run_phase(int layer, int phase, hipStream_t st) {
    if (!layer_ok(layer) || phase < 0 || phase > 2 || (phase == 1 && layer == 0)) return NITI_INVALID_VALUE;
    const bool t = tuning;
    tuning = false;
    std::unique_ptr<Collective> c = std::move(coll), cg = std::move(coll_grad);
    const int rc = phase == 0 ? fwd_layer(layer, st) : phase == 1 ? dgrad_layer(layer, st) : wgrad_layer(layer, st);
    coll = std::move(c);
    coll_grad = std::move(cg);
    tuning = t;
    return rc;
}

int Model::plan_info(int layer, int phase, int info[4]) {
    if (!layer_ok(layer) || phase < 0 || phase > 2) return NITI_INVALID_VALUE;
    const int op = plan_op(phase);
    PlanChoice c = conv_plan_query(op, L[layer].g, phase != 2, ws_bytes_for(op));
    if (phase == 2 && wgrad_p16_splits(layer) > 0) {
        c.bm = c.bn = PLAN_P16_TILE;
        c.splits = wgrad_p16_splits(layer);
        c.strat = c.splits > 1 ? 2 : 0;
    }
    return plan_out(c, info);
// ... 242 lines not shown
```

mandheling-dsp-training_amd/csrc/niti_wgrad.hip:

```cpp
#include <hip/hip_ext.h>

#include <algorithm>
#include <type_traits>

#include "niti_device.hpp"
#include "niti_kernels.hpp"

namespace niti {

struct WgP16 {
    const int8_t* x;
    const int8_t* dy;
    uint32_t xbytes, dybytes;
    int CIP, COP, c_out;
    int64_t ldc;
    int bpi;
    int kg_total, kg_per_split, kg_per_wave, splits;
    int tiles_ci, tiles;
    FastDiv fTiles, fTci;
    int32_t* C;
    uint32_t* amax;
    int32_t* slab;
    int64_t slab_stride;
    unsigned long long* span;
    unsigned long long* stamps;
};

constexpr int P16_TILE = 9 * 32 * 32;
constexpr int P16_WAVES = 4;

#ifndef NITI_WG_STAMPS
#define NITI_WG_STAMPS 0
#endif
#ifndef NITI_WG_ABLATE
#define NITI_WG_ABLATE 0
#endif
#ifndef NITI_WG_D8
#define NITI_WG_D8 4
#endif
#ifndef NITI_WG_D4
#define NITI_WG_D4 4
#endif
#ifndef NITI_WG_MERGE
#define NITI_WG_MERGE 1
#endif
#ifndef NITI_WG_NT_OUT
#define NITI_WG_NT_OUT 1
#endif
#ifndef NITI_WG_SWAP
#define NITI_WG_SWAP 1
#endif
#ifndef NITI_WG_ATOMIC_OUT
#define NITI_WG_ATOMIC_OUT 0
#endif
#define WG_WSTAMP(k)                                                                                       \
    do {                                                                                                   \
        if (NITI_WG_STAMPS && g.stamps != nullptr && (threadIdx.x & 63) == 0)                              \
            g.stamps[gridDim.x * 8 + (blockIdx.x * 4 + (threadIdx.x >> 6)) * 2 + (k)] = __builtin_amdgcn_s_memtime(); \
    } while (0)
#define WG_STAMP(k)                                                                            \
    do {                                                                                       \
        if (NITI_WG_STAMPS && g.stamps != nullptr && threadIdx.x == 0) {                        \
            g.stamps[blockIdx.x * 8 + (k)] = __builtin_amdgcn_s_memtime();                     \
            if ((k) == 0 || (k) == 5)                                                          \
                g.stamps[blockIdx.x * 8 + 6 + ((k) == 5)] = __builtin_amdgcn_s_memrealtime();  \
        }                                                                                      \
    } while (0)

__device__ __forceinline__ int ab(int hi, int lo, int s) {
    return (int)__builtin_amdgcn_alignbit((uint32_t)hi, (uint32_t)lo, (uint32_t)s);
}

template <int DY, int DX>
constexpr uint32_t perm2x2() {
    uint32_t s = 0;
    for (int i = 0; i < 4; ++i) {
        const int iy = (i >> 1) + DY, ix = (i & 1) + DX;
        const uint32_t b = (iy >= 0 && iy < 2 && ix >= 0 && ix < 2) ? (uint32_t)(2 * iy + ix) : 0x0cu;
        s |= b << (8 * i);
    }
    return s;
}

template <int OW, int KX>
__device__ __forceinline__ v4i dy_tap(v4i d) {
    if constexpr (KX == 1) {
        return d;
    } else if constexpr (OW == 8) {
        if constexpr (KX == 0)
            return v4i{ab(d[1], d[0], 8), (int)((uint32_t)d[1] >> 8), ab(d[3], d[2], 8), (int)((uint32_t)d[3] >> 8)};
        else
            return v4i{(int)((uint32_t)d[0] << 8), ab(d[1], d[0], 24), (int)((uint32_t)d[2] << 8), ab(d[3], d[2], 24)};
    } else if constexpr (OW == 16) {
        if constexpr (KX == 0)
            return v4i{ab(d[1], d[0], 8), ab(d[2], d[1], 8), ab(d[3], d[2], 8), (int)((uint32_t)d[3] >> 8)};
        else
            return v4i{(int)((uint32_t)d[0] << 8), ab(d[1], d[0], 24), ab(d[2], d[1], 24), ab(d[3], d[2], 24)};
    } else if constexpr (OW == 4) {
        v4i r;
#pragma unroll
        for (int i = 0; i < 4; ++i) r[i] = KX == 0 ? (int)((uint32_t)d[i] >> 8) : (int)((uint32_t)d[i] << 8);
        return r;
    } else {
        constexpr uint32_t sel = perm2x2<0, 1 - KX>();
        v4i r;
#pragma unroll
        for (int i = 0; i < 4; ++i) r[i] = (int)__builtin_amdgcn_perm((uint32_t)d[i], (uint32_t)d[i], sel);
        return r;
    }
}

template <int OW, int KY>
__device__ __forceinline__ v4i x_tap(const v4i& up, const v4i& x, const v4i& dn) {
    if constexpr (KY == 1) {
        return x;
    } else if constexpr (OW == 8) {
        return KY == 0 ? v4i{up[0], up[1], x[0], x[1]} : v4i{x[2], x[3], dn[0], dn[1]};
    } else if constexpr (OW == 16) {
        return KY == 0 ? up : dn;
    } else if constexpr (OW == 4) {
        return KY == 0 ? v4i{0, x[0], x[1], x[2]} : v4i{x[1], x[2], x[3], 0};
    } else {
        constexpr uint32_t sel = perm2x2<KY - 1, 0>();
        v4i r;
#pragma unroll
        for (int i = 0; i < 4; ++i) r[i] = (int)__builtin_amdgcn_perm((uint32_t)x[i], (uint32_t)x[i], sel);
        return r;
    }
}

__device__ __forceinline__ v2i asm_load8(__amdgpu_buffer_rsrc_t r, uint32_t voff, uint32_t soff) {
    v2i v;
    asm volatile("buffer_load_dwordx2 %0, %1, %2, %3 offen" : "=v"(v) : "v"(voff), "s"(r), "s"(soff));
    return v;
}
__device__ __forceinline__ v4i asm_load16(__amdgpu_buffer_rsrc_t r, uint32_t voff, uint32_t soff) {
    v4i v;
    asm volatile("buffer_load_dwordx4 %0, %1, %2, %3 offen" : "=v"(v) : "v"(voff), "s"(r), "s"(soff));
    return v;
}

template <int OW, int NW, int D>
__global__ void __launch_bounds__(NW * 64) wgrad_p16_kernel(WgP16 g) {
    static_assert(D >= 2 && D % 2 == 0, "the next K group's window must be resident; operand buffers alternate");
    constexpr int SMEM = (NITI_WG_MERGE ? 4 * P16_TILE * 4 : P16_TILE * 4) + 64;
    __shared__ v4i lds4[SMEM / 16];
    int8_t* smem = (int8_t*)lds4;

    const int tid = threadIdx.x;
    const int lane = tid & 63;
    const int wid = __builtin_amdgcn_readfirstlane(tid >> 6);
    const unsigned long long span_t0 = span_begin(g.span);
    WG_STAMP(0);
    WG_WSTAMP(0);
    const int logical = xcd_remap(blockIdx.x, gridDim.x);
    const int split = (int)fdiv(g.fTiles, (uint32_t)logical);
    const int tile = logical - split * g.tiles;
    const int tco = (int)fdiv(g.fTci, (uint32_t)tile), tci = tile - tco * g.tiles_ci;
    const int co0 = tco * 32, ci0 = tci * 32;
    const int kg_begin = split * g.kg_per_split;
    const int kg_end = min(g.kg_total, kg_begin + g.kg_per_split);
    const int kb = kg_begin + wid * g.kg_per_wave;
    const int n_w = max(0, min(kg_end, kb + g.kg_per_wave) - kb);

    const __amdgpu_buffer_rsrc_t rX = make_rsrc(g.x, g.xbytes);
    const __amdgpu_buffer_rsrc_t rD = make_rsrc(g.dy, g.dybytes);
    const int h = lane >> 5, c = lane & 31;
    const uint32_t xrow = (uint32_t)g.CIP * 16u, drow = (uint32_t)g.COP * 16u;
    const uint32_t lx = (uint32_t)h * xrow + (uint32_t)(ci0 + c) * 16u;
    const uint32_t ld = (uint32_t)h * drow + (uint32_t)(co0 + c) * 16u;
    constexpr uint32_t OOBS = 0x80000000u;
    const uint32_t ci16 = (uint32_t)(ci0 + c) * 16u;

    v16i acc[9];
#pragma unroll
    for (int t = 0; t < 9; ++t)
#pragma unroll
        for (int i = 0; i < 16; ++i) acc[t][i] = 0;
    int32_t* tile_lds = (int32_t*)smem;
    if (!NITI_WG_MERGE)
        for (int e = tid; e < P16_TILE / 4; e += NW * 64) ((v4i*)tile_lds)[e] = v4i{0, 0, 0, 0};

    constexpr bool NB = OW == 8 || OW == 16;
    constexpr int KPI = OW == 8 ? 2 : OW == 16 ? 8 : 1;
    constexpr uint32_t UPOFF = OW == 8 ? 8u : 0u;
    constexpr int L = NB ? 4 : 2;
    static_assert(D % KPI == 0, "unrolled steps cover whole images");
    const uint32_t vup_first = h ? ci16 + UPOFF : OOB, vup = lx + UPOFF;
    const uint32_t vdn = lx + xrow, vdn_last = h ? OOB : lx + xrow;
    typedef typename std::conditional<OW == 8, v2i, v4i>::type Row;
    struct Ring {
        v4i d, x;
        Row up, dn;
    };
    Ring ring[D];
    auto issue = [&](Ring& r, auto u_c, int j) {
        constexpr int U = decltype(u_c)::value;
        const uint32_t sx = (uint32_t)(kb + j) * 2u * xrow;
        const uint32_t sd = j < n_w ? (uint32_t)(kb + j) * 2u * drow : OOBS;
        if (NITI_WG_ABLATE == 1) return;
        r.d = asm_load16(rD, ld, sd);
        r.x = asm_load16(rX, lx, sx);
        if constexpr (NB) {
            constexpr bool first = U % KPI == 0, last = U % KPI == KPI - 1;
            if constexpr (OW == 8) {
                r.up = first ? asm_load8(rX, vup_first, sx) : asm_load8(rX, vup, sx - xrow);
                r.dn = asm_load8(rX, last ? vdn_last : vdn, sx);
            } else {
                r.up = first ? asm_load16(rX, vup_first, sx) : asm_load16(rX, vup, sx - xrow);
                r.dn = asm_load16(rX, last ? vdn_last : vdn, sx);
            }
        }
    };
    [&]<int... U>(std::integer_sequence<int, U...>) {
        ((ring[U] = Ring{}, issue(ring[U], std::integral_constant<int, U>(), U)), ...);
    }(std::make_integer_sequence<int, D>());
    WG_STAMP(1);
    struct Ops {
        v4i a0, a2, b0, b2;
    };
    Ops ops[2];
    auto prep = [&](Ring& r, Ops& o) {
        reg_fence(r.d);
        reg_fence(r.x);
        if constexpr (NB) {
            reg_fence(r.up);
            reg_fence(r.dn);
        }
        v4i up{0, 0, 0, 0}, dn{0, 0, 0, 0};
        if constexpr (OW == 8) {
            up = v4i{r.up[0], r.up[1], 0, 0};
            dn = v4i{r.dn[0], r.dn[1], 0, 0};
        } else if constexpr (OW == 16) {
            up = r.up;
            dn = r.dn;
        }
        if constexpr (NITI_WG_ABLATE == 3) {
            o.a0 = o.a2 = r.d;
            o.b0 = o.b2 = r.x;
        } else {
            o.a0 = dy_tap<OW, 0>(r.d);
            o.a2 = dy_tap<OW, 2>(r.d);
            o.b0 = x_tap<OW, 0>(up, r.x, dn);
            o.b2 = x_tap<OW, 2>(up, r.x, dn);
        }
    };
    wait_vmcnt<L * (D - 1)>();
    prep(ring[0], ops[0]);
    auto step = [&](auto u_c, int j0) {
        constexpr int u = decltype(u_c)::value, un = (u + 1) % D;
        wait_vmcnt<L * (D - 2)>();
        prep(ring[un], ops[(u + 1) & 1]);
        const Ops& o = ops[u & 1];
        const v4i A[3] = {o.a0, ring[u].d, o.a2};
        const v4i B[3] = {o.b0, ring[u].x, o.b2};
        [&]<int... T>(std::integer_sequence<int, T...>) {
            (([&] {
                 constexpr int KY = T / 3, KX = T % 3;
                 if constexpr (NITI_WG_ABLATE == 2)
                     acc[T][0] += A[KX][0] ^ B[KY][1];
                 else if constexpr (NITI_WG_MERGE && NITI_WG_SWAP)
                     acc[T] = __builtin_amdgcn_mfma_i32_32x32x32_i8(B[KY], A[KX], acc[T], 0, 0, 0);
                 else
                     acc[T] = __builtin_amdgcn_mfma_i32_32x32x32_i8(A[KX], B[KY], acc[T], 0, 0, 0);
             }()),
             ...);
        }(std::make_integer_sequence<int, 9>());
        issue(ring[u], u_c, j0 + u + D);
    };
    for (int j0 = 0; j0 < n_w; j0 += D) {
        [&]<int... U>(std::integer_sequence<int, U...>) {
            (step(std::integral_constant<int, U>(), j0), ...);
        }(std::make_integer_sequence<int, D>());
    }
    asm volatile("s_waitcnt vmcnt(0)" ::: "memory");
#pragma unroll
    for (int u = 0; u < D; ++u) {
        reg_fence(ring[u].d);
        reg_fence(ring[u].x);
        if constexpr (NB) {
            reg_fence(ring[u].up);
            reg_fence(ring[u].dn);
        }
    }
    WG_STAMP(2);
    WG_WSTAMP(1);

    constexpr int THREADS = NW * 64;
    const bool partial = g.splits > 1;
    int32_t* dst = partial ? g.slab + (int64_t)split * g.slab_stride : g.C;
    uint32_t lmax = 0;
    uint32_t* red = (uint32_t*)(smem + SMEM - 64);
    if constexpr (NITI_WG_MERGE) {
        static_assert(NW == 4, "one accumulator row quarter per wave");
        if constexpr (NITI_WG_SWAP) {
#pragma unroll
            for (int q = 0; q < 4; ++q)
#pragma unroll
                for (int t = 0; t < 9; ++t)
                    lds4[((wid * 4 + q) * 9 + t) * 64 + (lane ^ (2 * q + (lane >> 5) + 8 * (q & 1)))] =
                        v4i{acc[t][4 * q], acc[t][4 * q + 1], acc[t][4 * q + 2], acc[t][4 * q + 3]};
            __syncthreads();
            WG_STAMP(3);
            const int r = lane >> 3, c = lane & 7, co = 8 * wid + r;
            const int pos = (co + 32 * (c & 1)) ^ (c + 8 * ((c >> 1) & 1)), q = c >> 1;
            v4i sum[9];
#pragma unroll
            for (int t = 0; t < 9; ++t) sum[t] = lds4[((0 * 4 + q) * 9 + t) * 64 + pos];
#pragma unroll
            for (int w = 1; w < 4; ++w)
#pragma unroll
                for (int t = 0; t < 9; ++t) sum[t] += lds4[((w * 4 + q) * 9 + t) * 64 + pos];
            WG_STAMP(4);
            if (co0 + co < g.c_out && NITI_WG_ABLATE != 5) {
                int32_t* o = dst + (int64_t)(co0 + co) * g.ldc + ci0 + 4 * c;
#pragma unroll
                for (int t = 0; t < 9; ++t) {
                    __builtin_nontemporal_store(sum[t], (v4i*)(o + t * g.CIP));
#pragma unroll
                    for (int j = 0; j < 4; ++j) {
                        const uint32_t u = uabs32(sum[t][j]);
                        lmax = lmax > u ? lmax : u;
                    }
                }
            }
        } else {
#pragma unroll
        for (int q = 0; q < 4; ++q)
            if (q != wid) {
#pragma unroll
                for (int t = 0; t < 9; ++t)
                    lds4[((wid * 4 + q) * 9 + t) * 64 + lane] =
                        v4i{acc[t][4 * q], acc[t][4 * q + 1], acc[t][4 * q + 2], acc[t][4 * q + 3]};
            }
        v4i sum[9];
        switch (wid) {
#define NITI_OWN(W)                                                                                          \
    case W:                                                                                                  \
        for (int t = 0; t < 9; ++t) sum[t] = v4i{acc[t][4 * W], acc[t][4 * W + 1], acc[t][4 * W + 2], acc[t][4 * W + 3]}; \
        break;
            NITI_OWN(0)
            NITI_OWN(1)
            NITI_OWN(2)
            default:
                NITI_OWN(3)
#undef NITI_OWN
        }
        __syncthreads();
        WG_STAMP(3);
#pragma unroll
        for (int k = 1; k < 4; ++k) {
            const int w = (wid + k) & 3;
#pragma unroll
            for (int t = 0; t < 9; ++t) sum[t] += lds4[((w * 4 + wid) * 9 + t) * 64 + lane];
        }
        WG_STAMP(4);
#pragma unroll
        for (int j = 0; j < 4; ++j) {
            const int row = 8 * wid + j + 4 * (lane >> 5);
            if (co0 + row < g.c_out && NITI_WG_ABLATE != 5) {
                int32_t* o = dst + (int64_t)(co0 + row) * g.ldc + ci0 + (lane & 31);
#pragma unroll
                for (int t = 0; t < 9; ++t) {
                    const int32_t v = sum[t][j];
                    __builtin_nontemporal_store(v, o + t * g.CIP);
                    const uint32_t u = uabs32(v);
                    lmax = lmax > u ? lmax : u;
                }
            }
        }
        }
    } else {
    __syncthreads();
    WG_STAMP(3);
#pragma unroll
    for (int t = 0; t < 9; ++t)
#pragma unroll
        for (int i = 0; i < 16; ++i) {
            const int row = (i & 3) + 8 * (i >> 2) + 4 * (lane >> 5);
            __hip_atomic_fetch_add(tile_lds + (row * 9 + t) * 32 + (lane & 31), acc[t][i], __ATOMIC_RELAXED,
                                   __HIP_MEMORY_SCOPE_WORKGROUP);
        }
    __syncthreads();
    WG_STAMP(4);

    for (int c = tid; c < P16_TILE / 4; c += THREADS) {
        const int row = c / 72, rem = c - row * 72, t = rem >> 3, c4 = rem & 7;
        const v4i v = ((const v4i*)tile_lds)[c];
        if (co0 + row < g.c_out && NITI_WG_ABLATE != 5) {
            if (NITI_WG_ATOMIC_OUT && partial) {
                int32_t* q = g.C + (int64_t)(co0 + row) * g.ldc + t * g.CIP + ci0 + 4 * c4;
#pragma unroll
                for (int e = 0; e < 4; ++e)
                    __hip_atomic_fetch_add(q + e, v[e], __ATOMIC_RELAXED, __HIP_MEMORY_SCOPE_AGENT);
            } else if (NITI_WG_NT_OUT) {
                __builtin_nontemporal_store(v, (v4i*)(dst + (int64_t)(co0 + row) * g.ldc + t * g.CIP + ci0 + 4 * c4));
            } else {
                *(v4i*)(dst + (int64_t)(co0 + row) * g.ldc + t * g.CIP + ci0 + 4 * c4) = v;
            }
#pragma unroll
            for (int e = 0; e < 4; ++e) {
                const uint32_t u = uabs32(v[e]);
                lmax = lmax > u ? lmax : u;
            }
        }
    }
    }
    if (!partial && g.amax != nullptr) {
        lmax = wave_max(lmax);
        if (lane == 0) red[wid] = lmax;
        __syncthreads();
        if (tid == 0) {
            uint32_t m = red[0];
            for (int w = 1; w < NW; ++w) m = m > red[w] ? m : red[w];
            publish_max(g.amax, m);
        }
    }
    if (NITI_WG_STAMPS) {
        asm volatile("s_waitcnt vmcnt(0)" ::: "memory");
        WG_STAMP(5);
    }
    span_end(g.span, span_t0);
}

__global__ void __launch_bounds__(256) nhwc16_to_p16_kernel(P16Jobs J) {
    __shared__ __attribute__((aligned(16))) int8_t tile[16 * 1024];
    p16_convert_block(J, blockIdx.x, tile);
}

__global__ void nhwc16_to_p16_any_kernel(const int8_t* __restrict__ in, int64_t blocks, int cp,
                                         int8_t* __restrict__ out) {
    const int64_t e = (int64_t)blockIdx.x * 256 + threadIdx.x;
    const int cc = cp / 16;
    if (e >= blocks * cc) return;
    const int64_t b = e / cc;
    const int c16 = (int)(e - b * cc);
    v16c px[16];
#pragma unroll
    for (int p = 0; p < 16; ++p) px[p] = *(const v16c*)(in + ((b * 16 + p) * cp + c16 * 16));
#pragma unroll
    for (int k = 0; k < 16; ++k) {
        v16c o;
#pragma unroll
        for (int p = 0; p < 16; ++p) o[p] = px[p][k];
        *(v16c*)(out + (b * cp + c16 * 16 + k) * 16) = o;
    }
}

hipError_t p16_jobs_build(const P16Conv* jobs, int n, hipStream_t st, P16Jobs* out, uint32_t* wgs_out) {
    if (n < 0 || n > P16_MAX_JOBS) return hipErrorInvalidValue;
    P16Jobs& J = *out;
    J = P16Jobs{};
    uint32_t wg = 0;
    for (int i = 0; i < n; ++i) {
        const P16Conv& c = jobs[i];
        if (c.cp <= 0 || c.cp % 16 != 0 || c.pixels < 0 || c.pixels % 16 != 0) return hipErrorInvalidValue;
        if (c.pixels == 0) continue;
        const int64_t blocks = c.pixels / 16;
        if ((c.cp & (c.cp - 1)) != 0 || c.cp < 32 || c.cp > 1024) {
            const int64_t t = blocks * (c.cp / 16);
            hipLaunchKernelGGL(nhwc16_to_p16_any_kernel, dim3((unsigned)((t + 255) / 256)), dim3(256), 0, st, c.in,
                               blocks, c.cp, c.out);
            continue;
        }
        int lg = 0;
        while ((1 << lg) < c.cp) ++lg;
        const int bpw = lg < 8 ? 1 << (8 - lg) : 1;
        const int64_t wgs = (blocks + bpw - 1) / bpw;
        if ((int64_t)wg + wgs > 0x7fffffff) return hipErrorInvalidValue;
        J.j[J.n++] = P16Job{c.in, c.out, blocks, lg, wg};
        wg += (uint32_t)wgs;
    }
    *wgs_out = wg;
    return hipGetLastError();
}

hipError_t nhwc16_to_p16_many(const P16Conv* jobs, int n, hipStream_t st) {
    P16Jobs J;
    uint32_t wg = 0;
    hipError_t e = p16_jobs_build(jobs, n, st, &J, &wg);
    if (e != hipSuccess) return e;
    if (J.n > 0) hipLaunchKernelGGL(nhwc16_to_p16_kernel, dim3(wg), dim3(256), 0, st, J);
    return hipGetLastError();
}

hipError_t nhwc16_to_p16(const int8_t* in, int64_t pixels, int cp, int8_t* out, hipStream_t st) {
    const P16Conv c{in, pixels, cp, out};
    return nhwc16_to_p16_many(&c, 1, st);
}

static unsigned long long* g_wg_stamps = nullptr;
void wgrad_stamps_arm(unsigned long long* buf) { g_wg_stamps = buf; }

static bool p16_geom(const ConvGeom& g, WgP16* t) {
    if (g.kh != 3 || g.kw != 3 || g.sh != 1 || g.sw != 1 || g.dh != 1 || g.dw != 1) return false;
    if (g.pt != 1 || g.pl != 1 || g.pb != 1 || g.pr != 1) return false;
    if (g.cip % 32 != 0 || g.cop % 32 != 0) return false;
    const int ow = g.ow, oh = g.oh;
    if (oh != ow || !(ow == 8 || ow == 16 || ow == 4 || ow == 2)) return false;
    const int64_t po = (int64_t)g.n * oh * ow;
    if (po % 32 != 0) return false;
    if (po * g.cip > 0x7fffffff || po * g.cop > 0x7fffffff) return false;
    WgP16 w{};
    w.CIP = g.cip;
    w.COP = g.cop;
// ... 9 lines not shown
    *t = w;
    return true;
}

bool conv_wgrad_p16_ok(const ConvGeom& g) {
    WgP16 t;
    return p16_geom(g, &t);
}

int conv_wgrad_p16_splits(const ConvGeom& g) {
    WgP16 t;
    if (!p16_geom(g, &t)) return 0;
    const int kpi = g.ow == 8 ? 2 : g.ow == 16 ? 8 : 1;
    int s = std::max(1, 256 / t.tiles);
    s = std::min(s, 8);
    s = std::min(s, std::max(1, t.kg_total / kpi));
    return s;
}

static int64_t p16_slab_stride(const ConvGeom& g) {
    const int64_t bytes = (int64_t)g.c_out * 9 * g.cip * 4;
    return ((bytes + 4095) / 4096 | 1) * 1024;
}

size_t conv_wgrad_p16_workspace(const ConvGeom& g, int splits) {
    WgP16 t;
    if (!p16_geom(g, &t)) return 0;
    if (splits <= 0) splits = conv_wgrad_p16_splits(g);
    return splits > 1 ? (size_t)splits * p16_slab_stride(g) * 4 : 0;
}

hipError_t conv_wgrad_p16(const ConvGeom& g, const int8_t* x_p16, const int8_t* dy_p16, int32_t* acc,
                          uint32_t* amax, void* ws, size_t ws_bytes, int splits, hipStream_t st, hipEvent_t ev_b,
                          hipEvent_t ev_e, unsigned long long* span, SgdJob* defer) {
    WgP16 t;
    if (!p16_geom(g, &t)) return hipErrorInvalidValue;
    if (splits <= 0) splits = conv_wgrad_p16_splits(g);
    if (splits < 1 || splits > 64) return hipErrorInvalidValue;
    t.x = x_p16;
    t.dy = dy_p16;
    const int kpi = g.ow == 8 ? 2 : g.ow == 16 ? 8 : 1;
    auto round_kpi = [&](int v) { return (v + kpi - 1) / kpi * kpi; };
    t.kg_per_split = round_kpi((t.kg_total + splits - 1) / splits);
    t.splits = (t.kg_total + t.kg_per_split - 1) / t.kg_per_split;
    t.kg_per_wave = round_kpi((t.kg_per_split + P16_WAVES - 1) / P16_WAVES);
    if (t.splits > 1 && (ws == nullptr || ws_bytes < (size_t)t.splits * p16_slab_stride(g) * 4))
        return hipErrorInvalidValue;
    t.fTiles = make_fastdiv((uint32_t)t.tiles);
    t.C = acc;
    t.amax = amax;
    t.slab = (int32_t*)ws;
    t.slab_stride = p16_slab_stride(g);
    t.span = span;
    t.stamps = g_wg_stamps;
    constexpr int NW = P16_WAVES;
    const dim3 grid((unsigned)(t.tiles * t.splits));
    auto launch = [&](auto k) {
        if (ev_b != nullptr && ev_e != nullptr)
            hipExtLaunchKernelGGL(k, grid, dim3(NW * 64), 0, st, ev_b, ev_e, 0, t);
        else
            hipLaunchKernelGGL(k, grid, dim3(NW * 64), 0, st, t);
    };
    switch (g.ow) {
        case 8: launch(wgrad_p16_kernel<8, NW, NITI_WG_D8>); break;
        case 16: launch(wgrad_p16_kernel<16, NW, 8>); break;
        case 4: launch(wgrad_p16_kernel<4, NW, NITI_WG_D4>); break;
        default: launch(wgrad_p16_kernel<2, NW, NITI_WG_D4>); break;
    }
    hipError_t e = hipGetLastError();
    if (e == hipSuccess && t.splits > 1) {
        const int64_t n = (int64_t)g.c_out * 9 * g.cip;
        if (defer != nullptr) {
            defer->slab = t.slab;
            defer->splits = t.splits;
            defer->slab_stride = t.slab_stride;
            defer->slab_n = n;
        } else {
            e = splitk_reduce_linear(t.slab, t.splits, n, t.slab_stride, acc, amax, st);
        }
    }
    return e;
}

}
```

mandheling-dsp-training_amd/niti_amd/_lib.py:

```python
from __future__ import annotations

import ctypes as C
import os
import re

_HERE = os.path.dirname(os.path.abspath(__file__))
LIB_PATH = os.environ.get("NITI_HIP_LIB") or os.path.join(_HERE, "_lib", "libniti_hip.so")
HEADER = os.path.join(os.path.dirname(os.path.dirname(_HERE)), "include", "niti_hip.h")

ERROR_NAMES = {0: "NO_ERROR", 1: "OUT_OF_MEMORY", 2: "NOT_SUPPORT", 3: "COMPUTE_SIZE_ERROR",
               4: "NO_EXECUTION", 5: "INVALID_VALUE", 10: "INPUT_DATA_ERROR", 11: "CALL_BACK_STOP"}

OP_CONV_INT8 = 700
OP_DECONV_INT8 = 701
OP_RELU_INT8 = 703
OP_RELUGRAD_INT8 = 704
OP_MAXPOOL_INT8 = 705
OP_POOLGRAD_INT8 = 706
OP_LOSS_INT8 = 710
OP_LOSS_GRAD_INT8 = 711
OP_MATMUL_INT8 = 713
OP_PAD_INT8 = 714
OP_LEFTPOOLGRAD_INT8 = 718
OP_GRADIENT_CONV_INT8 = 715
OP_DSP_CONV_INT8 = 800
OP_DSP_RELU_INT8 = 801
OP_DSP_MAXPOOL_INT8 = 802
OP_DSP_RESHAPE_INT8 = 803
OP_DSP_LOSSGRAD_INT8 = 804
OP_DSP_RELUGRAD_INT8 = 805
OP_DSP_MAXPOOLGRAD_INT8 = 807
OP_DSP_TRANSPOSE_INT8 = 808
OP_DSP_WEIGHTROTATE180_INT8 = 809
OP_DSP_RESHAPEGRAD_INT8 = 813
OP_DSP_LEFTPOOLGRAD_DECONV_INT8 = 814
OP_DSP_LEFTPOOLGRAD_GRADIENT_INT8 = 815
OP_DSP_NOP_INT8 = 817
OP_DSP_DECONV_INT8 = 811
OP_DSP_MATMUL_GRADIENT_INT8 = 818
OP_DSP_PARALLEL_GRADIENTCONV_INT8 = 820
OP_DSP_GRADIENT_SPLITBATCHCONV_INT8 = 821
OP_DSP_TRANSPOSEGRADIENT_CONV_INT8 = 822
FORMAT_NCHW, FORMAT_NHWC, FORMAT_NC4HW4 = 0, 1, 2
PAD_CAFFE, PAD_VALID, PAD_SAME = 0, 1, 2
ARCH_LENET, ARCH_VGG11, ARCH_VGG16, ARCH_RESNET18 = 1, 2, 3, 4


class NitiError(RuntimeError):
    def __init__(self, code, what=""):
        self.code = code
        super().__init__(f"{what}: {ERROR_NAMES.get(code, code)}")


class Tensor(C.Structure):
    _fields_ = [("data", C.c_void_p), ("dims", C.c_int * 4), ("format", C.c_int)]


class ConvCommon(C.Structure):
    _fields_ = [("kernel_x", C.c_int), ("kernel_y", C.c_int), ("stride_x", C.c_int), ("stride_y", C.c_int),
                ("dilate_x", C.c_int), ("dilate_y", C.c_int), ("pad_x", C.c_int), ("pad_y", C.c_int),
                ("has_pads", C.c_int), ("pads", C.c_int * 4), ("pad_mode", C.c_int),
                ("input_count", C.c_int), ("output_count", C.c_int), ("group", C.c_int)]


class Geom(C.Structure):
    _fields_ = [(n, C.c_int) for n in (
        "n", "c_in", "h", "w", "c_out", "kh", "kw", "stride_h", "stride_w", "pad_t", "pad_l", "pad_b",
        "pad_r", "dilate_h", "dilate_w", "oh", "ow", "cip", "cop", "np")]


class EvalTotals(C.Structure):
    _fields_ = [("images", C.c_uint64), ("top1", C.c_uint64), ("topk", C.c_uint64), ("loss_sum", C.c_double)]


class RequantFused(C.Structure):
    _fields_ = ([(n, C.c_void_p) for n in (
        "exp_in", "wscale", "exp_out", "relu_mask", "out_nhwc16", "pool_out", "pool_x", "pool_y", "pool_dx",
        "pool_dx_c32", "out_p16", "pool3_out", "pool3_arg")] + [(n, C.c_int) for n in (
            "relu", "pool_relu", "pool_h", "pool_w", "zero_cls", "zc_h", "zc_w", "pool3_h", "pool3_w", "pool3_oh",
            "pool3_ow")])


_lib = None


def header_functions():
    src = open(HEADER).read()
    src = re.sub(r"/\*.*?\*/", "", src, flags=re.S)
    return sorted(set(re.findall(r"^\s*(?:const\s+)?[a-z_0-9]+\*?\s+\*?(niti_[a-z0-9_]+)\s*\(", src, flags=re.M)))


def lib():
    global _lib
    if _lib is not None:
        return _lib
    if not os.path.exists(LIB_PATH):
        raise ImportError(f"libniti_hip.so not built ({LIB_PATH}); run __graft_entry__.build() or "
                          f"make -C mandheling-dsp-training_amd/csrc")
    import torch
    L = C.CDLL(LIB_PATH)
    vp, i32, i64, ci = C.c_void_p, C.c_int32, C.c_int64, C.c_int
    tp = C.POINTER(Tensor)
    sig = {
        "niti_version": (C.c_char_p, []),
        "niti_create_execution": (ci, [ci, C.POINTER(ConvCommon), C.POINTER(vp)]),
        "niti_execution_resize": (ci, [vp, tp, ci, tp, ci]),
        "niti_execution_execute": (ci, [vp, tp, ci, tp, ci, vp]),
        "niti_destroy_execution": (None, [vp]),
        "niti_execution_workspace_bytes": (C.c_size_t, [vp]),
        "niti_execution_status": (ci, [vp, vp]),
        "niti_diag_rowconv_barrier": (None, [C.c_uint32, C.c_uint32]),
        "niti_diag_rowconv_speculate": (None, [C.c_int]),
        "niti_diag_gemm_speculate": (None, [C.c_int]),
        "niti_diag_gemm_fused_launches": (C.c_ulonglong, []),
        "niti_diag_head_chain_launches": (C.c_ulonglong, []),
        "niti_diag_head_chain": (None, [C.c_int]),
        "niti_diag_p16_jobs_cap": (None, [C.c_int]),
        "niti_tensor_convert": (ci, [tp, tp, vp]),
        "niti_geom_finalize": (ci, [C.POINTER(Geom)]),
        "niti_conv_workspace_bytes": (ci, [C.POINTER(Geom), ci, C.POINTER(C.c_size_t)]),
        "niti_matmul_workspace_bytes": (ci, [ci, ci, ci, C.POINTER(C.c_size_t)]),
        "niti_conv_plan_info": (ci, [C.POINTER(Geom), ci, C.c_size_t, C.POINTER(C.c_int)]),
        "niti_conv_fwd_acc": (ci, [C.POINTER(Geom), vp, vp, vp, vp, vp, C.c_size_t, vp]),
        "niti_conv_dgrad_acc": (ci, [C.POINTER(Geom), vp, vp, vp, vp, vp, C.c_size_t, vp]),
        "niti_conv_wgrad_acc": (ci, [C.POINTER(Geom), vp, vp, vp, vp, vp, C.c_size_t, vp]),
        "niti_conv_fwd_phase1": (ci, [C.POINTER(Geom), vp, vp, vp, vp, vp, C.c_size_t, vp]),
        "niti_conv_rows_ok": (ci, [C.POINTER(Geom)]),
        "niti_nhwc16_to_c32": (ci, [vp, ci, ci, ci, ci, vp, vp]),
        "niti_weights_to_wf": (ci, [vp, ci, ci, ci, ci, vp, vp]),
        "niti_conv_fwd_rows": (ci, [C.POINTER(Geom), vp, vp, vp, vp, vp, ci, vp, vp, vp, ci, vp, vp, C.c_uint32, vp,
                                    vp]),
        "niti_conv_dgrad_rows": (ci, [C.POINTER(Geom), vp, vp, vp, vp, vp, ci, vp, vp, vp, vp, vp, vp, ci, vp, vp, C.c_uint32, vp, vp]),
        "niti_rows_spec_slot": (vp, [vp, ci]),
        "niti_conv_fwd_phase2": (ci, [C.POINTER(Geom), vp, vp, vp, vp, vp, vp, vp, ci, vp, vp, C.c_size_t, vp]),
        "niti_conv_dgrad_phase1": (ci, [C.POINTER(Geom), vp, vp, vp, vp, vp, C.c_size_t, vp]),
        "niti_conv_dgrad_phase2": (ci, [C.POINTER(Geom), vp, vp, vp, vp, vp, vp, vp, ci, vp, vp, C.c_size_t, vp]),
        "niti_nhwc16_to_p16": (ci, [vp, i64, ci, vp, vp]),
        "niti_diag_wgrad_stamps": (None, [vp]),
        "niti_diag_rowconv_stamps": (None, [vp]),
        "niti_conv_wgrad_p16_workspace": (ci, [C.POINTER(Geom), ci, C.POINTER(C.c_size_t)]),
        "niti_conv_wgrad_p16_acc": (ci, [C.POINTER(Geom), vp, vp, vp, vp, vp, C.c_size_t, ci, vp]),
        "niti_matmul_acc": (ci, [ci, ci, ci, vp, i64, vp, i64, vp, i64, vp, vp, C.c_size_t, vp]),
        "niti_absmax_i32": (ci, [vp, i64, vp, vp]),
        "niti_requant_act": (ci, [vp, i64, ci, vp, vp, vp, vp, ci, vp, vp, vp]),
        "niti_requant_act_fused": (ci, [vp, i64, ci, vp, C.POINTER(RequantFused), vp]),
        "niti_requant_grad": (ci, [vp, i64, vp, ci, vp, vp, vp]),
        "niti_sgd_update": (ci, [vp, vp, ci, ci, ci, ci, ci, ci, vp, vp, vp, vp]),
        "niti_nhwc16_to_chwn16": (ci, [vp, ci, ci, ci, ci, vp, vp]),
        "niti_ohwi16_to_ihwo16": (ci, [vp, ci, ci, ci, ci, ci, vp, vp]),
        "niti_nchw_to_nhwc16": (ci, [vp, ci, ci, ci, ci, vp, vp]),
        "niti_nchw_to_chwn16": (ci, [vp, ci, ci, ci, ci, ci, vp, vp]),
        "niti_nhwc16_to_nchw": (ci, [vp, ci, ci, ci, ci, vp, vp]),
        "niti_oihw_to_ohwi16": (ci, [vp, ci, ci, ci, ci, vp, vp]),
        "niti_ohwi16_to_oihw": (ci, [vp, ci, ci, ci, ci, vp, vp]),
        "niti_residual_add": (ci, [vp, vp, vp, vp, i64, vp, vp, vp, vp]),
        "niti_residual_requant": (ci, [vp, vp, vp, vp, i64, vp, vp, vp, ci, vp, vp]),
        "niti_residual_requant_relu_grad": (ci, [vp, vp, vp, vp, i64, vp, vp, vp, vp, vp, vp]),
        "niti_sum_pool": (ci, [vp, ci, ci, ci, vp, vp, vp]),
        "niti_sum_pool_grad": (ci, [vp, ci, ci, ci, vp, vp]),
        "niti_im2col": (ci, [C.POINTER(Geom), vp, ci, vp, vp]),
        "niti_im2col_nchw": (ci, [C.POINTER(Geom), vp, ci, vp, vp]),
        "niti_sgd_update_wf": (ci, [vp, vp, ci, ci, ci, ci, ci, ci, vp, vp, vp, vp, vp, vp]),
        "niti_conv_rows_nhwc_ok": (ci, [C.POINTER(Geom), ci]),
        "niti_conv_plan_set": (ci, [C.POINTER(Geom), ci, vp]),
        "niti_maxpool": (ci, [vp] + [ci] * 7 + [vp, ci, ci, vp]),
        "niti_maxpool_grad": (ci, [vp, vp, vp] + [ci] * 10 + [vp, vp]),
        "niti_maxpool_grad_ws": (ci, [vp, vp, vp] + [ci] * 10 + [vp, vp, vp]),
        "niti_maxpool_arg": (ci, [vp] + [ci] * 7 + [vp, ci, ci, vp, vp]),
        "niti_maxpool_grad_arg": (ci, [vp, vp, vp] + [ci] * 10 + [vp, vp, vp]),
        "niti_relu_grad": (ci, [vp, vp, i64, vp, vp]),
        "niti_loss_grad": (ci, [vp, ci, ci, ci, vp, vp, vp, vp]),
        "niti_head_metrics": (ci, [vp, ci, ci, ci, vp, vp, ci, vp, vp, vp, vp, C.c_size_t, vp]),
        "niti_head_metrics_workspace": (ci, [ci, C.POINTER(C.c_size_t)]),
        "niti_model_eval_step": (ci, [vp, vp, ci, vp, vp]),
        "niti_model_eval_step_images": (ci, [vp, vp, vp, vp]),
        "niti_model_eval_reset": (ci, [vp, vp]),
        "niti_model_eval_read": (ci, [vp, C.POINTER(EvalTotals), vp]),
        "niti_model_eval_topk": (ci, [vp, ci]),
        "niti_model_get_predictions": (ci, [vp, vp, vp]),
        "niti_model_copy_weights": (ci, [vp, vp, vp]),
        "niti_model_create": (ci, [ci, ci, C.POINTER(vp)]),
        "niti_model_create2": (ci, [ci, ci, ci, C.POINTER(vp)]),
        "niti_model_create3": (ci, [ci, ci, ci, ci, C.POINTER(vp)]),
        "niti_model_destroy": (None, [vp]),
        "niti_model_num_layers": (ci, [vp]),
        "niti_model_layer_info": (ci, [vp, ci, C.POINTER(ci)]),
        "niti_model_set_weight": (ci, [vp, ci, vp, ci]),
        "niti_model_get_weight": (ci, [vp, ci, vp]),
        "niti_model_train_step": (ci, [vp, vp, ci, vp, vp]),
        "niti_model_get_logits": (ci, [vp, vp, C.POINTER(ci), vp]),
        "niti_model_get_tap": (ci, [vp, ci, ci, vp, C.c_size_t, vp]),
        "niti_model_step_macs": (i64, [vp]),
        "niti_model_set_graph": (ci, [vp, ci]),
        "niti_model_set_rowconv": (ci, [vp, ci]),
        "niti_model_keep_grads": (ci, [vp, ci]),
        "niti_model_rowconv_error": (ci, [vp]),
        "niti_model_spec_stats": (ci, [vp, vp, ci]),
        "niti_model_autotune": (ci, [vp, ci, vp]),
        "niti_model_set_overlap": (ci, [vp, ci]),
        "niti_model_plan_info": (ci, [vp, ci, ci, C.POINTER(ci)]),
        "niti_model_plan_set": (ci, [vp, ci, ci, C.POINTER(ci)]),
        "niti_plan_reset": (None, []),
        "niti_model_set_probe": (ci, [vp, ci, ci, ci]),
        "niti_model_probe_read": (ci, [vp, C.POINTER(C.c_double), C.POINTER(ci)]),
        "niti_model_probe_pause": (ci, [vp, ci]),
        "niti_model_spec_slot": (ci, [vp, ci, ci, C.POINTER(C.c_uint32)]),
        "niti_model_run_phase": (ci, [vp, ci, ci, vp]),
        "niti_model_probe_read_span": (ci, [vp, C.POINTER(C.c_double), C.POINTER(ci)]),
        "niti_dp_get_unique_id": (ci, [C.c_char_p]),
        "niti_model_attach_comm": (ci, [vp, C.c_char_p, ci, ci, ci]),
        "niti_image_stats": (ci, [vp, i64, vp, vp]),
        "niti_image_quantize": (ci, [vp, ci, ci, ci, vp, i64, vp, vp, vp]),
        "niti_image_quantize_nhwc16": (ci, [vp, ci, ci, ci, ci, vp, i64, vp, vp, vp]),
        "niti_model_train_step_images": (ci, [vp, vp, vp, vp]),
        "niti_model_get_input": (ci, [vp, vp, C.POINTER(ci), vp]),
        "niti_dataset_create": (ci, [vp, vp, i64, ci, ci, ci, C.POINTER(vp)]),
        "niti_dataset_destroy": (None, [vp]),
        "niti_dataset_order_check": (ci, [vp, vp, i64, i64, ci, ci]),
        "niti_dataset_set_order": (ci, [vp, vp, vp, i64]),
        "niti_dataset_set_output": (ci, [vp, ci, ci]),
        "niti_dataset_windows_check": (ci, [vp, vp, i64, ci, ci]),
        "niti_dataset_set_order_windows": (ci, [vp, vp, vp, vp, i64]),
        "niti_batch_gather": (ci, [vp, i64, ci, vp, vp, vp]),
        "niti_model_train_steps_dataset": (ci, [vp, vp, i64, ci, vp]),
# ... 20 lines not shown
```

mandheling-dsp-training_amd/niti_amd/ops.py:

```python
from __future__ import annotations

import ctypes as C

import torch

from . import _lib as L
from ._lib import check


def _stream(stream=None):
    if stream is not None:
        return stream
    return C.c_void_p(torch.cuda.current_stream().cuda_stream)


def _ptr(t):
    return None if t is None else C.c_void_p(t.data_ptr())


def tensor(t: torch.Tensor, dims, fmt=L.FORMAT_NCHW) -> L.Tensor:
    d = list(dims) + [1] * (4 - len(dims))
    v = L.Tensor(t.data_ptr(), (C.c_int * 4)(*d), fmt)
    v._keep = t
    return v
# ... 243 lines not shown
                    pool_x=None, pool_y=None, pool_relu=False, dx_c32=False, dx_p16=False, exp_in=None, wscale=None,
                    exp_out=None, x_nhwc=False, stream=None, outs=None):
    dev = dyc32.device
    hh, ww = (2 * g.h, 2 * g.w) if pool_x is not None else (g.h, g.w)
    if outs is not None:
        dx, nxt, p16 = outs
    else:
        dx = None if mode == 1 else torch.empty((g.n, hh, ww, g.cip), dtype=torch.int8, device=dev)
        nxt = torch.empty((g.n, g.cip // 32, hh, ww, 32), dtype=torch.int8, device=dev) if dx_c32 and mode != 1 else None
        p16 = torch.empty((g.n * hh * ww // 16, g.cip, 16), dtype=torch.int8, device=dev) if dx_p16 and mode != 1 else None
    st_ptr = err_ptr = None
    epoch = 0
    if mode == 0:
        epoch, st_ptr, err_ptr = state.epoch + 1, _ptr(state.state), _ptr(state.err)
    elif mode >= 3:
        st_ptr = _ptr(state.state)
    check(L.lib().niti_conv_dgrad_rows(C.byref(g), _ptr(dyc32), _ptr(wft), _ptr(relu_mask), _ptr(pool_x),
                                       _ptr(pool_y), 1 if pool_relu else 0, _ptr(dx), _ptr(nxt), _ptr(p16),
                                       _ptr(exp_in), _ptr(wscale), _ptr(exp_out),
                                       mode | (ROWS_X_NHWC16 if x_nhwc else 0),
                                       _ptr(amax), st_ptr, epoch, err_ptr, _stream(stream)), "conv_dgrad_rows")
    if mode == 0:
        state.epoch = epoch
    return dx, nxt, p16


def conv_fwd_requant(g: L.Geom, x16, w16, amax, exp_in=None, wscale=None, exp_out=None, relu=False,
                     relu_mask=None, between=None, stream=None):
    return _conv_requant(0, g, x16, w16, amax, exp_in, wscale, exp_out, relu, relu_mask, between, stream)


def conv_dgrad_requant(g: L.Geom, dy16, wt16, amax, exp_in=None, wscale=None, exp_out=None, relu=False,
                       relu_mask=None, between=None, stream=None):
    return _conv_requant(1, g, dy16, wt16, amax, exp_in, wscale, exp_out, relu, relu_mask, between, stream)


def conv_plan(g: L.Geom, op: int, ws_bytes: int | None = None):
    if ws_bytes is None:
        n = C.c_size_t(0)
        check(L.lib().niti_conv_workspace_bytes(C.byref(g), op, C.byref(n)), "workspace")
        ws_bytes = int(n.value)
    info = (C.c_int * 4)()
    check(L.lib().niti_conv_plan_info(C.byref(g), op, ws_bytes, info), "conv_plan_info")
    return tuple(info)


def wgrad_taps_ok(g: L.Geom) -> bool:
    return conv_plan(g, 2)[0] == 32


def conv_wgrad_acc(g: L.Geom, xT, dyT, amax=None, stream=None):
    acc = torch.empty((g.c_out, g.kh, g.kw, g.cip), dtype=torch.int32, device=xT.device)
    ws, nb = conv_workspace(g, 2, xT.device)
    check(L.lib().niti_conv_wgrad_acc(C.byref(g), _ptr(xT), _ptr(dyT), _ptr(acc), _ptr(amax), _ptr(ws), nb,
                                      _stream(stream)), "conv_wgrad_acc")
    return acc


def nhwc16_to_p16(x16: torch.Tensor, stream=None):
    cp = x16.shape[-1]
    px = x16.numel() // cp
    out = torch.empty((px // 16, cp, 16), dtype=torch.int8, device=x16.device)
    check(L.lib().niti_nhwc16_to_p16(_ptr(x16), px, cp, _ptr(out), _stream(stream)), "nhwc16->p16")
    return out


def wgrad_p16_workspace(g: L.Geom, splits: int = 0, device="cuda"):
    n = C.c_size_t()
    check(L.lib().niti_conv_wgrad_p16_workspace(C.byref(g), splits, C.byref(n)), "p16 workspace")
    return torch.zeros(max(int(n.value), 16), dtype=torch.uint8, device=device), int(n.value)


def conv_wgrad_p16_acc(g: L.Geom, xP, dyP, amax=None, splits: int = 0, ws=None, stream=None):
    acc = torch.zeros((g.c_out, g.kh, g.kw, g.cip), dtype=torch.int32, device=xP.device)
    if ws is None:
        ws, nb = wgrad_p16_workspace(g, splits, xP.device)
    else:
        nb = ws.numel()
    check(L.lib().niti_conv_wgrad_p16_acc(C.byref(g), _ptr(xP), _ptr(dyP), _ptr(acc), _ptr(amax), _ptr(ws), nb,
                                          splits, _stream(stream)), "conv_wgrad_p16_acc")
    return acc


def matmul_acc(B16, A16, ldc, amax=None, use_workspace=True, stream=None):
    m, k16 = B16.shape
    o = A16.shape[0]
    acc = torch.empty((m, ldc), dtype=torch.int32, device=B16.device)
    n = C.c_size_t(0)
    if use_workspace:
        check(L.lib().niti_matmul_workspace_bytes(m, ldc, k16, C.byref(n)), "workspace")
    ws = torch.empty(max(int(n.value), 16), dtype=torch.uint8, device=B16.device)
    check(L.lib().niti_matmul_acc(m, o, k16, _ptr(B16), k16, _ptr(A16), k16, _ptr(acc), ldc, _ptr(amax), _ptr(ws),
                                  int(n.value), _stream(stream)), "matmul_acc")
    return acc


MAX_WORDS = 2048


def new_range(device="cuda"):
    return torch.zeros(MAX_WORDS, dtype=torch.int32, device=device)


def range_max(amax) -> int:
    return int(amax.view(-1, MAX_WORDS).max(dim=1).values.max().item())


def absmax(acc, amax, stream=None):
    check(L.lib().niti_absmax_i32(_ptr(acc), acc.numel(), _ptr(amax), _stream(stream)), "absmax")


def requant_act(acc, amax, exp_in=None, wscale=None, exp_out=None, relu=False, relu_mask=None, stream=None):
    rows, ldc = acc.shape
    out = torch.empty((rows, ldc), dtype=torch.int8, device=acc.device)
    check(L.lib().niti_requant_act(_ptr(acc), rows, ldc, _ptr(amax), _ptr(exp_in), _ptr(wscale), _ptr(exp_out),
                                   1 if relu else 0, _ptr(relu_mask), _ptr(out), _stream(stream)), "requant_act")
    return out


def requant_act_fused(acc, amax, *, exp_in=None, wscale=None, exp_out=None, relu=False, relu_mask=None, out=None,
                      pool_out=None, pool_x=None, pool_y=None, pool_dx=None, pool_relu=False, pool_hw=(0, 0),
                      pool_dx_c32=None, out_p16=None, zero_cls=0, zc_hw=(0, 0), pool3_out=None, pool3_arg=None,
                      pool3_hw=(0, 0), pool3_ohw=(0, 0), stream=None):
    rows, ldc = acc.shape
    f = L.RequantFused()
    for name, t in (("exp_in", exp_in), ("wscale", wscale), ("exp_out", exp_out), ("relu_mask", relu_mask),
                    ("out_nhwc16", out), ("pool_out", pool_out), ("pool_x", pool_x), ("pool_y", pool_y),
                    ("pool_dx", pool_dx), ("pool_dx_c32", pool_dx_c32), ("out_p16", out_p16),
                    ("pool3_out", pool3_out), ("pool3_arg", pool3_arg)):
        setattr(f, name, None if t is None else t.data_ptr())
    f.relu, f.pool_relu = (1 if relu else 0), (1 if pool_relu else 0)
    f.pool_h, f.pool_w = pool_hw
    f.zero_cls = zero_cls
    f.zc_h, f.zc_w = zc_hw
    f.pool3_h, f.pool3_w = pool3_hw
    f.pool3_oh, f.pool3_ow = pool3_ohw
    check(L.lib().niti_requant_act_fused(_ptr(acc), rows, ldc, _ptr(amax), C.byref(f), _stream(stream)),
          "requant_act_fused")


def requant_grad(acc, amax, rule=2, w_update=None, stream=None):
    g = torch.empty(acc.shape, dtype=torch.int8, device=acc.device)
    check(L.lib().niti_requant_grad(_ptr(acc), acc.numel(), _ptr(amax), rule, _ptr(g), _ptr(w_update),
                                    _stream(stream)), "requant_grad")
    return g


def sgd_update(acc, amax, w16, ci, rule=2, stream=None, wT=None, g=None, wf=None, wft=None):
    co, kh, kw, cip = acc.shape
    cop = r16(co)
    if wT is None:
        wT = torch.zeros((ci, kh, kw, cop), dtype=torch.int8, device=acc.device)
    if g is None:
        g = torch.empty(acc.shape, dtype=torch.int8, device=acc.device)
    assert wT.shape == (ci, kh, kw, cop) and g.shape == acc.shape
    if wf is not None or wft is not None:
        check(L.lib().niti_sgd_update_wf(_ptr(acc), _ptr(amax), rule, co, ci, kh * kw, cip, cop, _ptr(w16), _ptr(wT),
                                         _ptr(g), _ptr(wf), _ptr(wft), _stream(stream)), "sgd_update_wf")
        return wT, g
    check(L.lib().niti_sgd_update(_ptr(acc), _ptr(amax), rule, co, ci, kh * kw, cip, cop, _ptr(w16), _ptr(wT), _ptr(g),
                                  _stream(stream)), "sgd_update")
    return wT, g


def residual_add(a, ea, b, eb, amax, stream=None, ez=None):
    assert a.shape == b.shape and a.dtype == b.dtype == torch.int8
# ... 173 lines not shown
```

Baseline: 690,600 images/s.

## Batch all p16 conv weight-gradient layers into one load-balanced persistent launch

```diff
diff --git a/include/niti_hip.h b/include/niti_hip.h
--- a/include/niti_hip.h
+++ b/include/niti_hip.h
@@ -150,6 +150,18 @@
 void niti_diag_p16_jobs_cap(int cap);
 int niti_conv_wgrad_p16_acc(const niti_geom* g, const int8_t* x_p16, const int8_t* dy_p16, int32_t* acc,
                             uint32_t* amax, void* workspace, size_t workspace_bytes, int splits, void* stream);
+typedef struct niti_wgrad_p16_job {
+    niti_geom g;
+    const int8_t* x_p16;
+    const int8_t* dy_p16;
+    int32_t* acc;
+    uint32_t* amax;
+} niti_wgrad_p16_job;
+int niti_conv_wgrad_p16_many_workspace(const niti_wgrad_p16_job* jobs, int n, int blocks, int t, size_t* bytes);
+int niti_conv_wgrad_p16_many(const niti_wgrad_p16_job* jobs, int n, int blocks, int t, void* workspace,
+                             size_t workspace_bytes, int* splits_out, void* stream);
+void niti_diag_wgrad_batch(int mode);
+unsigned long long niti_diag_wgrad_batch_launches(void);
 int niti_matmul_acc(int m, int o, int k16, const int8_t* B, int64_t ldb, const int8_t* A, int64_t lda,
                     int32_t* acc, int64_t ldc, uint32_t* amax, void* workspace, size_t workspace_bytes,
                     void* stream);
diff --git a/mandheling-dsp-training_amd/csrc/niti_capi.hip b/mandheling-dsp-training_amd/csrc/niti_capi.hip
--- a/mandheling-dsp-training_amd/csrc/niti_capi.hip
+++ b/mandheling-dsp-training_amd/csrc/niti_capi.hip
@@ -473,6 +473,64 @@
     if (ws_bytes < niti::conv_wgrad_p16_workspace(r, splits) || (ws_bytes > 0 && !ws)) return NITI_INVALID_VALUE;
     return code(niti::conv_wgrad_p16(r, x, dy, acc, amax, ws, ws_bytes, splits, S(stream)));
 }
+
+static int p16_many_jobs(const niti_wgrad_p16_job* jobs, int n, int blocks, int t, unsigned char* ws,
+                         niti::WgP16Job* out, niti::WgP16Many* m, size_t* table_room, size_t* bytes) {
+    if (!jobs || n < 1 || n > niti::P16_MANY_MAX_JOBS || blocks < 1 || t < 1) return NITI_INVALID_VALUE;
+    for (int pass = 0; pass < 2; ++pass) {
+        size_t off = *table_room;
+        for (int j = 0; j < n; ++j) {
+            niti::WgP16Job& o = out[j];
+            if (!to_geom(&jobs[j].g, &o.g)) return NITI_COMPUTE_SIZE_ERROR;
+            if (!niti::conv_wgrad_p16_ok(o.g)) return NITI_NOT_SUPPORT;
+            if (!jobs[j].x_p16 || !jobs[j].dy_p16 || !jobs[j].acc) return NITI_INVALID_VALUE;
+            o.x_p16 = jobs[j].x_p16;
+            o.dy_p16 = jobs[j].dy_p16;
+            o.acc = jobs[j].acc;
+            o.amax = jobs[j].amax;
+            o.slab_bytes = niti::conv_wgrad_p16_workspace(o.g, 8);
+            o.slab = (int32_t*)(ws + off);
+            off += o.slab_bytes;
+        }
+        if (niti::conv_wgrad_p16_many_build(out, n, blocks, t, m) != hipSuccess) return NITI_INVALID_VALUE;
+        *bytes = off;
+        if (pass == 0) *table_room = (m->table_bytes + 4095) / 4096 * 4096;
+    }
+    return NITI_NO_ERROR;
+}
+
+int niti_conv_wgrad_p16_many_workspace(const niti_wgrad_p16_job* jobs, int n, int blocks, int t, size_t* bytes) {
+    if (!bytes) return NITI_INVALID_VALUE;
+    niti::WgP16Job r[niti::P16_MANY_MAX_JOBS];
+    niti::WgP16Many m;
+    size_t room = 4096;
+    return p16_many_jobs(jobs, n, blocks, t, (unsigned char*)(uintptr_t)4096, r, &m, &room, bytes);
+}
+
+int niti_conv_wgrad_p16_many(const niti_wgrad_p16_job* jobs, int n, int blocks, int t, void* ws, size_t ws_bytes,
+                             int* splits_out, void* stream) {
+    if (!ws) return NITI_INVALID_VALUE;
+    niti::WgP16Job r[niti::P16_MANY_MAX_JOBS];
+    niti::WgP16Many m;
+    size_t room = 4096, need = 0;
+    if (const int rc = p16_many_jobs(jobs, n, blocks, t, (unsigned char*)ws, r, &m, &room, &need)) return rc;
+    if (ws_bytes < need) return NITI_INVALID_VALUE;
+    hipStream_t st = S(stream);
+    if (hipMemcpyAsync(ws, m.table, m.table_bytes, hipMemcpyHostToDevice, st) != hipSuccess ||
+        hipStreamSynchronize(st) != hipSuccess)
+        return NITI_NO_EXECUTION;
+    hipError_t e = niti::conv_wgrad_p16_many(m, ws, st);
+    for (int j = 0; j < n && e == hipSuccess; ++j) {
+        if (splits_out) splits_out[j] = m.splits[j];
+        if (m.splits[j] > 1)
+            e = niti::splitk_reduce_linear(r[j].slab, m.splits[j], (int64_t)r[j].g.c_out * 9 * r[j].g.cip,
+                                           m.slab_stride[j], r[j].acc, r[j].amax, st);
+    }
+    return code(e);
+}
+
+void niti_diag_wgrad_batch(int mode) { niti::model_wgrad_batch(mode); }
+unsigned long long niti_diag_wgrad_batch_launches(void) { return niti::conv_wgrad_p16_many_launches(); }
 
 int niti_matmul_acc(int m, int o, int k16, const int8_t* B, int64_t ldb, const int8_t* A, int64_t lda, int32_t* acc,
                     int64_t ldc, uint32_t* amax, void* ws, size_t ws_bytes, void* stream) {
diff --git a/mandheling-dsp-training_amd/csrc/niti_kernels.hip b/mandheling-dsp-training_amd/csrc/niti_kernels.hip
--- a/mandheling-dsp-training_amd/csrc/niti_kernels.hip
+++ b/mandheling-dsp-training_amd/csrc/niti_kernels.hip
@@ -3776,6 +3776,25 @@
     }
 }
 
+hipError_t sgd_combine_many(const SgdJob* jobs, int n, hipStream_t st) {
+    if (n <= 0) return hipSuccess;
+    if (n > SGD_MAX_JOBS) return hipErrorInvalidValue;
+    SgdJobs J{};
+    J.n = n;
+    int chunks = 0;
+    for (int i = 0; i < n; ++i) {
+        J.job[i] = jobs[i];
+        J.cstart[i] = chunks;
+        if (jobs[i].slab != nullptr) {
+            if (jobs[i].splits < 1 || jobs[i].slab_stride % 4 != 0 || jobs[i].slab_n % 4 != 0) return hipErrorInvalidValue;
+            chunks += (int)((jobs[i].slab_n + 1023) / 1024);
+        }
+    }
+    J.cstart[n] = chunks;
+    if (chunks > 0) hipLaunchKernelGGL(sgd_combine_kernel, dim3(chunks < 2048 ? chunks : 2048), dim3(256), 0, st, J);
+    return hipGetLastError();
+}
+
 hipError_t sgd_update_many(const SgdJob* jobs, int n, hipStream_t st) {
     if (n <= 0) return hipSuccess;
     if (n > SGD_MAX_JOBS) return hipErrorInvalidValue;
diff --git a/mandheling-dsp-training_amd/csrc/niti_kernels.hpp b/mandheling-dsp-training_amd/csrc/niti_kernels.hpp
--- a/mandheling-dsp-training_amd/csrc/niti_kernels.hpp
+++ b/mandheling-dsp-training_amd/csrc/niti_kernels.hpp
@@ -106,6 +106,37 @@
                           uint32_t* amax, void* ws, size_t ws_bytes, int splits, hipStream_t st,
                           hipEvent_t ev_b = nullptr, hipEvent_t ev_e = nullptr, unsigned long long* span = nullptr,
                           SgdJob* defer = nullptr);
+struct WgP16Job {
+    ConvGeom g;
+    const int8_t* x_p16 = nullptr;
+    const int8_t* dy_p16 = nullptr;
+    int32_t* acc = nullptr;
+    uint32_t* amax = nullptr;
+    int32_t* slab = nullptr;
+    size_t slab_bytes = 0;
+};
+constexpr int P16_MANY_MAX_JOBS = 16;
+struct WgP16Many {
+    unsigned char* table = nullptr;
+    size_t table_bytes = 0, starts_off = 0, items_off = 0;
+    int blocks = 0, n_jobs = 0, n_items = 0;
+    int splits[P16_MANY_MAX_JOBS] = {};
+    int64_t slab_stride[P16_MANY_MAX_JOBS] = {};
+    int max_list_kg = 0;
+    WgP16Many() = default;
+    WgP16Many(const WgP16Many&) = delete;
+    WgP16Many& operator=(const WgP16Many&) = delete;
+    void clear() {
+        free(table);
+        table = nullptr;
+        table_bytes = 0;
+        n_jobs = n_items = blocks = 0;
+    }
+    ~WgP16Many() { clear(); }
+};
+hipError_t conv_wgrad_p16_many_build(const WgP16Job* jobs, int n, int blocks, int t, WgP16Many* out);
+hipError_t conv_wgrad_p16_many(const WgP16Many& m, const void* table_dev, hipStream_t st);
+unsigned long long conv_wgrad_p16_many_launches();
 hipError_t matmul_acc(int M, int O, int k16, const int8_t* B, int64_t ldb, const int8_t* A, int64_t lda,
                       int32_t* acc, int64_t ldc, uint32_t* amax, void* ws, size_t ws_bytes, hipStream_t st);
 
@@ -225,6 +256,7 @@
 void rowconv_speculate(int mode);
 uint32_t* rowconv_spec_slot(uint32_t* bar, bool dg);
 void model_p16_jobs_cap(int cap);
+void model_wgrad_batch(int mode);
 hipError_t rowconv_fwd(const ConvGeom& g, const int8_t* x_c32, const int8_t* wf, const RowConvOut& o, int mode,
                        uint32_t* amax, uint32_t* bar, uint32_t epoch, uint32_t* err, hipStream_t st);
 struct HeadChain {
@@ -324,6 +356,7 @@
     int n;
 };
 hipError_t sgd_update_many(const SgdJob* jobs, int n, hipStream_t st);
+hipError_t sgd_combine_many(const SgdJob* jobs, int n, hipStream_t st);
 bool conv_wgrad_fc_sgd_ok(const ConvGeom& g);
 hipError_t conv_wgrad_fc_sgd(const ConvGeom& g, const int8_t* x, const int8_t* dy, uint32_t* amax, const SgdJob& j,
                              int pass, hipStream_t st);
diff --git a/mandheling-dsp-training_amd/csrc/niti_model.hip b/mandheling-dsp-training_amd/csrc/niti_model.hip
--- a/mandheling-dsp-training_amd/csrc/niti_model.hip
+++ b/mandheling-dsp-training_amd/csrc/niti_model.hip
@@ -13,8 +13,10 @@
 
 namespace {
 extern int g_p16_jobs_cap;
+extern int g_wgrad_batch;
 }
 void model_p16_jobs_cap(int cap) { g_p16_jobs_cap = cap <= 0 ? P16_MAX_JOBS : cap; }
+void model_wgrad_batch(int mode) { g_wgrad_batch = mode < 0 ? 1 : mode; }
 
 namespace {
 
@@ -61,6 +63,8 @@
 };
 
 int g_p16_jobs_cap = P16_MAX_JOBS;
+int g_wgrad_batch = getenv("NITI_WGRAD_BATCH") != nullptr ? std::max(0, atoi(getenv("NITI_WGRAD_BATCH"))) : 1;
+constexpr int WGRAD_BATCH_T = 256;
 
 static hipError_t im2col32(const ConvGeom& o, const int8_t* x16, int8_t* out, hipStream_t st) {
     const int64_t px = (int64_t)o.n * o.oh * o.ow;
@@ -352,6 +356,7 @@
         return !keep && i - 1 >= 1 && next != nullptr && p16 != nullptr && wgrad_p16_splits(i - 1) > 0;
     }
     int autotune(hipStream_t st, int reps) override;
+    int tune_wgrad_batch(hipStream_t st, TuneTimer& timer, bool log);
     size_t ws_bytes_for(int op) const { return op == PLAN_WGRAD ? slab_w_bytes : slab_bytes; }
     bool ensure_wslab(int i) const {
         const Layer& l = L[i];
@@ -376,6 +381,88 @@
             if (!p) return NITI_OUT_OF_MEMORY;
         }
         wslab_epoch = plan_override_epoch();
+        return NITI_NO_ERROR;
+    }
+    int wgb_tuned = WGRAD_BATCH_T;
+    WgP16Many wgb;
+    std::vector<int> wgb_layers;
+    void* wgb_dev = nullptr;
+    size_t wgb_dev_bytes = 0;
+    unsigned wgb_epoch = 0;
+    int wgb_t = -1, wgb_probe = -2;
+    int wgrad_batch_t() const {
+        if (dp() || g_wgrad_batch == 0) return 0;
+        return g_wgrad_batch == 1 ? wgb_tuned : g_wgrad_batch;
+    }
+    int build_wgrad_batch(int t) {
+        const int pl = probe_phase == 2 ? probe_layer : -1;
+        if (wgb_t == t && wgb_probe == pl && wgb_epoch == plan_override_epoch()) return NITI_NO_ERROR;
+        drop_graph();
+        wgb.clear();
+        wgb_layers.clear();
+        wgb_t = t;
+        wgb_probe = pl;
+        wgb_epoch = plan_override_epoch();
+        if (t <= 0) return NITI_NO_ERROR;
+        WgP16Job jobs[P16_MANY_MAX_JOBS];
+        std::vector<int> layers;
+        for (int i = 0; i < (int)L.size(); ++i) {
+            if (wgrad_p16_splits(i) <= 0 || i == pl) continue;
+            if ((int)layers.size() == P16_MANY_MAX_JOBS) return NITI_NO_ERROR;
+            Layer& l = L[i];
+            WgP16Job& j = jobs[layers.size()];
+            j.g = l.g;
+            j.x_p16 = xp16[i];
+            j.dy_p16 = dp16[i];
+            j.acc = l.dwacc;
+            j.amax = rng(i, 2);
+            j.slab = l.slab16;
+            j.slab_bytes = l.slab16_bytes;
+            layers.push_back(i);
+        }
+        if (layers.size() < 2) return NITI_NO_ERROR;
+        int cus = 0, dev = 0;
+        if (hipGetDevice(&dev) != hipSuccess ||
+            hipDeviceGetAttribute(&cus, hipDeviceAttributeMultiprocessorCount, dev) != hipSuccess || cus < 1)
+            return NITI_NO_EXECUTION;
+        if (conv_wgrad_p16_many_build(jobs, (int)layers.size(), cus, t, &wgb) != hipSuccess) return NITI_NO_EXECUTION;
+        if (hipDeviceSynchronize() != hipSuccess) return NITI_NO_EXECUTION;
+        if (wgb.table_bytes > wgb_dev_bytes) {
+            wgb_dev = ws.replace(wgb_dev, wgb.table_bytes);
+            wgb_dev_bytes = wgb_dev ? wgb.table_bytes : 0;
+            if (!wgb_dev) {
+                wgb.clear();
+                return NITI_OUT_OF_MEMORY;
+            }
+        }
+        if (hipMemcpy(wgb_dev, wgb.table, wgb.table_bytes, hipMemcpyHostToDevice) != hipSuccess) {
+            wgb.clear();
+            return NITI_NO_EXECUTION;
+        }
+        wgb_layers = layers;
+        return NITI_NO_ERROR;
+    }
+    bool wgrad_batched(int i) const {
+        return std::find(wgb_layers.begin(), wgb_layers.end(), i) != wgb_layers.end();
+    }
+    int wgrad_batch_run(bool defer, hipStream_t st) {
+        DTRY(conv_wgrad_p16_many(wgb, wgb_dev, st));
+        for (size_t k = 0; k < wgb_layers.size(); ++k) {
+            Layer& l = L[wgb_layers[k]];
+            l.defer = SgdJob{};
+            l.fc_sgd = false;
+            if (wgb.splits[k] < 2) continue;
+            const int64_t n = (int64_t)l.g.c_out * 9 * l.g.cip;
+            if (defer) {
+                l.defer.slab = l.slab16;
+                l.defer.splits = wgb.splits[k];
+                l.defer.slab_stride = wgb.slab_stride[k];
+                l.defer.slab_n = n;
+            } else {
+                DTRY(splitk_reduce_linear(l.slab16, wgb.splits[k], n, wgb.slab_stride[k], l.dwacc,
+                                          rng(wgb_layers[k], 2), st));
+            }
+        }
         return NITI_NO_ERROR;
     }
     int ensure_streams() {
@@ -644,6 +731,7 @@
 }
 
 int Model::step(const int8_t* x_nchw, int exp_in, const uint8_t* images, const int32_t* labels, hipStream_t st) {
+    if (const int rc = build_wgrad_batch(wgrad_batch_t())) return rc;
     if (!use_graph || coll != nullptr) return run(x_nchw, exp_in, images, labels, st);
     Key k;
     k.x = x_nchw ? (const void*)x_nchw : (const void*)images;
@@ -1098,9 +1186,77 @@
             if (rc != NITI_NO_ERROR) break;
         }
     }
+    if (rc == NITI_NO_ERROR) rc = tune_wgrad_batch(st, timer, log);
     invalidate_xp16();
     tuning = false;
     if (hipStreamSynchronize(st) != hipSuccess) rc = NITI_NO_EXECUTION;
+    return rc;
+}
+
+int Model::tune_wgrad_batch(hipStream_t st, TuneTimer& timer, bool log) {
+    if (dp() || g_wgrad_batch == 0) return NITI_NO_ERROR;
+    std::vector<int> set;
+    for (int i = 0; i < (int)L.size(); ++i)
+        if (wgrad_p16_splits(i) > 0 && !(probe_phase == 2 && probe_layer == i)) set.push_back(i);
+    if (set.size() < 2 || set.size() > (size_t)P16_MANY_MAX_JOBS) return NITI_NO_ERROR;
+    if (const int rc = convert_p16_inputs(st)) return rc;
+    for (int i : set)
+        if (!dp16_valid[i]) {
+            const ConvGeom& g = L[i].g;
+            DTRY(nhwc16_to_p16(L[i].dy, (int64_t)g.n * g.oh * g.ow, g.cop, dp16[i], st));
+            dp16_valid[i] = 1;
+        }
+    auto combine = [&]() -> int {
+        SgdJob jobs[SGD_MAX_JOBS];
+        int n = 0;
+        for (int i : set) {
+            Layer& l = L[i];
+            if (l.defer.slab == nullptr) continue;
+            jobs[n] = l.defer;
+            jobs[n].acc = l.dwacc;
+            jobs[n].amax = rng(i, 2);
+            ++n;
+            l.defer = SgdJob{};
+        }
+        return sgd_combine_many(jobs, n, st) == hipSuccess ? NITI_NO_ERROR : NITI_NO_EXECUTION;
+    };
+    auto per_layer = [&]() -> int {
+        for (int i : set) {
+            Layer& l = L[i];
+            const ConvGeom& g = l.g;
+            const int s = wgrad_p16_splits(i);
+            const bool defer = s > 1 && l.slab16 != nullptr && conv_wgrad_p16_workspace(g, s) <= l.slab16_bytes;
+            l.defer = SgdJob{};
+            DTRY(conv_wgrad_p16(g, xp16[i], dp16[i], l.dwacc, rng(i, 2), defer ? l.slab16 : slab_w,
+                                defer ? l.slab16_bytes : slab_w_bytes, s, st, nullptr, nullptr, nullptr,
+                                defer ? &l.defer : nullptr));
+        }
+        return combine();
+    };
+    auto batched = [&]() -> int {
+        if (const int rc = wgrad_batch_run(true, st)) return rc;
+        return combine();
+    };
+    float best_us = 0.f;
+    int best_t = 0;
+    int rc = timer.time(per_layer, &best_us);
+    if (log) fprintf(stderr, "tune wgrad set: per layer %.2f us\n", best_us);
+    for (int t : {128, 256, 512}) {
+        if (rc != NITI_NO_ERROR) break;
+        rc = build_wgrad_batch(t);
+        if (rc != NITI_NO_ERROR || wgb_layers.empty()) break;
+        float us = 0.f;
+        rc = timer.time(batched, &us);
+        if (log)
+            fprintf(stderr, "tune wgrad set: batch t %d (%d items, longest list %d K groups) %.2f us\n", t, wgb.n_items,
+                    wgb.max_list_kg, us);
+        if (rc == NITI_NO_ERROR && us < best_us) {
+            best_us = us;
+            best_t = t;
+        }
+    }
+    if (rc == NITI_NO_ERROR) wgb_tuned = best_t;
+    if (log) fprintf(stderr, "tune wgrad set: keeps %d\n", wgb_tuned);
     return rc;
 }
 
@@ -1254,6 +1410,21 @@
         if (rc != NITI_NO_ERROR) return rc;
     }
     hipStream_t wst = ov ? side : st;
+    const bool wbatch = !dp && !ov && !tuning && !wgb_layers.empty();
+    auto take_defer = [&](int i) {
+        const Layer& l = L[i];
+        if (l.defer.slab == nullptr) return;
+        jobs[i].slab = l.defer.slab;
+        jobs[i].splits = l.defer.splits;
+        jobs[i].slab_stride = l.defer.slab_stride;
+        jobs[i].slab_n = l.defer.slab_n;
+        jobs[i].slab_map = l.defer.slab_map;
+        jobs[i].tb_tiles_ci = l.defer.tb_tiles_ci;
+        jobs[i].tb_cip4 = l.defer.tb_cip4;
+        jobs[i].tb_ld4 = l.defer.tb_ld4;
+        jobs[i].tb_m = l.defer.tb_m;
+        jobs[i].tb_s = l.defer.tb_s;
+    };
     for (int i = nl - 1; i >= 0; --i) {
         if (ov) {
             DTRY(hipEventRecord(ev_dy[i], st));
@@ -1266,7 +1437,7 @@
         Layer& l = L[i];
         const ConvGeom& g = l.g;
         const bool in_chain = hc && i == nl - 1;
-        int rc = in_chain ? NITI_NO_ERROR : wgrad_layer(i, wst);
+        int rc = in_chain || (wbatch && wgrad_batched(i)) ? NITI_NO_ERROR : wgrad_layer(i, wst);
         if (rc == NITI_NO_ERROR && dp && closes_bucket[i]) rc = sum_bucket(i, wst);
         if (rc == NITI_NO_ERROR && i > 0 && !in_chain) rc = dgrad_layer(i, st);
         if (rc != NITI_NO_ERROR) return rc;
@@ -1274,18 +1445,22 @@
                          i > 0 && !rowconv_dgrad_layer(i) ? l.wT : nullptr, keep_grads ? l.g8 : nullptr};
         jobs[i].wf = l.rc ? l.wf : nullptr;
         jobs[i].wft = l.rcd ? l.wft : nullptr;
-        if (l.defer.slab != nullptr) {
-            jobs[i].slab = l.defer.slab;
-            jobs[i].splits = l.defer.splits;
-            jobs[i].slab_stride = l.defer.slab_stride;
-            jobs[i].slab_n = l.defer.slab_n;
-            jobs[i].slab_map = l.defer.slab_map;
-            jobs[i].tb_tiles_ci = l.defer.tb_tiles_ci;
-            jobs[i].tb_cip4 = l.defer.tb_cip4;
-            jobs[i].tb_ld4 = l.defer.tb_ld4;
-            jobs[i].tb_m = l.defer.tb_m;
-            jobs[i].tb_s = l.defer.tb_s;
-        }
+        take_defer(i);
+    }
+    if (wbatch) {
+        P16Conv cv[P16_MAX_JOBS];
+        int nc = 0;
+        for (int i : wgb_layers)
+            if (!dp16_valid[i]) {
+                const ConvGeom& g = L[i].g;
+                cv[nc++] = P16Conv{L[i].dy, (int64_t)g.n * g.oh * g.ow, g.cop, dp16[i]};
+                dp16_valid[i] = 1;
+            }
+        static_assert(P16_MANY_MAX_JOBS <= P16_MAX_JOBS, "one conversion launch holds every member");
+        if (nc > 0) DTRY(nhwc16_to_p16_many(cv, nc, st));
+        const int rc = wgrad_batch_run(defer_combine(), st);
+        if (rc != NITI_NO_ERROR) return rc;
+        for (int i : wgb_layers) take_defer(i);
     }
     if (dp) {
         DTRY(hipEventRecord(ev_grads, cst));
diff --git a/mandheling-dsp-training_amd/csrc/niti_wgrad.hip b/mandheling-dsp-training_amd/csrc/niti_wgrad.hip
--- a/mandheling-dsp-training_amd/csrc/niti_wgrad.hip
+++ b/mandheling-dsp-training_amd/csrc/niti_wgrad.hip
@@ -1,7 +1,11 @@
 #include <hip/hip_ext.h>
 
+#include <string.h>
+
 #include <algorithm>
+#include <atomic>
 #include <type_traits>
+#include <vector>
 
 #include "niti_device.hpp"
 #include "niti_kernels.hpp"
@@ -140,28 +144,24 @@
     return v;
 }
 
+constexpr int P16_SMEM = (NITI_WG_MERGE ? 4 * P16_TILE * 4 : P16_TILE * 4) + 64;
+
 template <int OW, int NW, int D>
-__global__ void __launch_bounds__(NW * 64) wgrad_p16_kernel(WgP16 g) {
+__device__ __forceinline__ void wgrad_p16_item(const WgP16& g, int tile, int slab, int kg_begin, int kg_end,
+                                               int kg_per_wave, v4i* lds4) {
     static_assert(D >= 2 && D % 2 == 0, "the next K group's window must be resident; operand buffers alternate");
-    constexpr int SMEM = (NITI_WG_MERGE ? 4 * P16_TILE * 4 : P16_TILE * 4) + 64;
-    __shared__ v4i lds4[SMEM / 16];
+    constexpr int SMEM = P16_SMEM;
     int8_t* smem = (int8_t*)lds4;
 
     const int tid = threadIdx.x;
     const int lane = tid & 63;
     const int wid = __builtin_amdgcn_readfirstlane(tid >> 6);
-    const unsigned long long span_t0 = span_begin(g.span);
     WG_STAMP(0);
     WG_WSTAMP(0);
-    const int logical = xcd_remap(blockIdx.x, gridDim.x);
-    const int split = (int)fdiv(g.fTiles, (uint32_t)logical);
-    const int tile = logical - split * g.tiles;
     const int tco = (int)fdiv(g.fTci, (uint32_t)tile), tci = tile - tco * g.tiles_ci;
     const int co0 = tco * 32, ci0 = tci * 32;
-    const int kg_begin = split * g.kg_per_split;
-    const int kg_end = min(g.kg_total, kg_begin + g.kg_per_split);
-    const int kb = kg_begin + wid * g.kg_per_wave;
-    const int n_w = max(0, min(kg_end, kb + g.kg_per_wave) - kb);
+    const int kb = kg_begin + wid * kg_per_wave;
+    const int n_w = max(0, min(kg_end, kb + kg_per_wave) - kb);
 
     const __amdgpu_buffer_rsrc_t rX = make_rsrc(g.x, g.xbytes);
     const __amdgpu_buffer_rsrc_t rD = make_rsrc(g.dy, g.dybytes);
@@ -287,8 +287,8 @@
     WG_WSTAMP(1);
 
     constexpr int THREADS = NW * 64;
-    const bool partial = g.splits > 1;
-    int32_t* dst = partial ? g.slab + (int64_t)split * g.slab_stride : g.C;
+    const bool partial = slab >= 0;
+    int32_t* dst = partial ? g.slab + (int64_t)slab * g.slab_stride : g.C;
     uint32_t lmax = 0;
     uint32_t* red = (uint32_t*)(smem + SMEM - 64);
     if constexpr (NITI_WG_MERGE) {
@@ -420,7 +420,50 @@
         asm volatile("s_waitcnt vmcnt(0)" ::: "memory");
         WG_STAMP(5);
     }
+}
+
+template <int OW, int NW, int D>
+__global__ void __launch_bounds__(NW * 64) wgrad_p16_kernel(WgP16 g) {
+    __shared__ v4i lds4[P16_SMEM / 16];
+    const unsigned long long span_t0 = span_begin(g.span);
+    const int logical = xcd_remap(blockIdx.x, gridDim.x);
+    const int split = (int)fdiv(g.fTiles, (uint32_t)logical);
+    const int tile = logical - split * g.tiles;
+    const int kg_begin = split * g.kg_per_split;
+    const int kg_end = min(g.kg_total, kg_begin + g.kg_per_split);
+    wgrad_p16_item<OW, NW, D>(g, tile, g.splits > 1 ? split : -1, kg_begin, kg_end, g.kg_per_wave, lds4);
     span_end(g.span, span_t0);
+}
+
+struct WgP16Desc {
+    WgP16 g;
+    int ow, pad;
+};
+struct WgP16Item {
+    int job, tile, slab, kg_begin, kg_end, kg_per_wave, pad0, pad1;
+};
+template <int NW>
+__global__ void __launch_bounds__(NW * 64) wgrad_p16_many_kernel(const WgP16Desc* __restrict__ descs,
+                                                                  const int* __restrict__ starts,
+                                                                  const WgP16Item* __restrict__ items) {
+    __shared__ v4i lds4[P16_SMEM / 16];
+    const int i0 = starts[blockIdx.x], i1 = starts[blockIdx.x + 1];
+    for (int i = i0; i < i1; ++i) {
+        const int job = __builtin_amdgcn_readfirstlane(items[i].job);
+        const int tile = __builtin_amdgcn_readfirstlane(items[i].tile);
+        const int slab = __builtin_amdgcn_readfirstlane(items[i].slab);
+        const int kg_begin = __builtin_amdgcn_readfirstlane(items[i].kg_begin);
+        const int kg_end = __builtin_amdgcn_readfirstlane(items[i].kg_end);
+        const int kpw = __builtin_amdgcn_readfirstlane(items[i].kg_per_wave);
+        const WgP16 g = descs[job].g;
+        switch (__builtin_amdgcn_readfirstlane(descs[job].ow)) {
+            case 8: wgrad_p16_item<8, NW, NITI_WG_D8>(g, tile, slab, kg_begin, kg_end, kpw, lds4); break;
+            case 16: wgrad_p16_item<16, NW, 8>(g, tile, slab, kg_begin, kg_end, kpw, lds4); break;
+            case 4: wgrad_p16_item<4, NW, NITI_WG_D4>(g, tile, slab, kg_begin, kg_end, kpw, lds4); break;
+            default: wgrad_p16_item<2, NW, NITI_WG_D4>(g, tile, slab, kg_begin, kg_end, kpw, lds4); break;
+        }
+        __syncthreads();
+    }
 }
 
 __global__ void __launch_bounds__(256) nhwc16_to_p16_kernel(P16Jobs J) {
@@ -596,4 +639,99 @@
     return e;
 }
 
-}
+constexpr int P16_ITEM_FIXED = 20;
+
+hipError_t conv_wgrad_p16_many_build(const WgP16Job* jobs, int n, int blocks, int t, WgP16Many* out) {
+    out->clear();
+    if (jobs == nullptr || n < 1 || n > P16_MANY_MAX_JOBS || blocks < 1 || blocks > 4096 || t < 1)
+        return hipErrorInvalidValue;
+    std::vector<WgP16Desc> descs((size_t)n);
+    std::vector<WgP16Item> items;
+    for (int j = 0; j < n; ++j) {
+        const WgP16Job& jb = jobs[j];
+        const ConvGeom& g = jb.g;
+        WgP16 w;
+        if (!p16_geom(g, &w) || !jb.x_p16 || !jb.dy_p16 || !jb.acc) return hipErrorInvalidValue;
+        const int kpi = g.ow == 8 ? 2 : g.ow == 16 ? 8 : 1;
+        auto round_kpi = [&](int v) { return (v + kpi - 1) / kpi * kpi; };
+        const int64_t stride = p16_slab_stride(g);
+        const int64_t room = jb.slab != nullptr ? (int64_t)(jb.slab_bytes / ((size_t)stride * 4)) : 0;
+        int s = std::max(1, (w.kg_total + t / 2) / t);
+        s = std::min(s, std::max(1, w.kg_total / kpi));
+        s = (int)std::min<int64_t>(std::min(s, 64), room >= 2 ? room : 1);
+        const int kg_per_split = round_kpi((w.kg_total + s - 1) / s);
+        s = (w.kg_total + kg_per_split - 1) / kg_per_split;
+        w.x = jb.x_p16;
+        w.dy = jb.dy_p16;
+        w.kg_per_split = kg_per_split;
+        w.kg_per_wave = round_kpi((kg_per_split + P16_WAVES - 1) / P16_WAVES);
+        w.splits = s;
+        w.fTiles = make_fastdiv((uint32_t)w.tiles);
+        w.C = jb.acc;
+        w.amax = jb.amax;
+        w.slab = s > 1 ? jb.slab : nullptr;
+        w.slab_stride = stride;
+        w.span = nullptr;
+        w.stamps = nullptr;
+        descs[j] = WgP16Desc{w, g.ow, 0};
+        out->splits[j] = s;
+        out->slab_stride[j] = stride;
+        for (int sp = 0; sp < s; ++sp) {
+            const int kb = sp * kg_per_split, ke = std::min(w.kg_total, kb + kg_per_split);
+            const int kpw = round_kpi((ke - kb + P16_WAVES - 1) / P16_WAVES);
+            for (int tile = 0; tile < w.tiles; ++tile)
+                items.push_back(WgP16Item{j, tile, s > 1 ? sp : -1, kb, ke, kpw, 0, 0});
+        }
+    }
+    std::vector<int> order(items.size());
+    for (size_t i = 0; i < order.size(); ++i) order[i] = (int)i;
+    auto len = [&](int i) { return items[i].kg_end - items[i].kg_begin; };
+    std::stable_sort(order.begin(), order.end(), [&](int a, int b) { return len(a) > len(b); });
+    std::vector<int64_t> load((size_t)blocks, 0);
+    std::vector<int> kg((size_t)blocks, 0);
+    std::vector<std::vector<int>> lists((size_t)blocks);
+    for (int i : order) {
+        const int b = (int)(std::min_element(load.begin(), load.end()) - load.begin());
+        lists[b].push_back(i);
+        load[b] += len(i) + P16_ITEM_FIXED;
+        kg[b] += len(i);
+    }
+    const size_t starts_off = (descs.size() * sizeof(WgP16Desc) + 63) / 64 * 64;
+    const size_t items_off = (starts_off + (size_t)(blocks + 1) * sizeof(int) + 63) / 64 * 64;
+    const size_t bytes = items_off + items.size() * sizeof(WgP16Item);
+    unsigned char* tb = (unsigned char*)calloc(bytes, 1);
+    if (tb == nullptr) return hipErrorOutOfMemory;
+    memcpy(tb, descs.data(), descs.size() * sizeof(WgP16Desc));
+    int* starts = (int*)(tb + starts_off);
+    WgP16Item* it = (WgP16Item*)(tb + items_off);
+    int k = 0;
+    for (int b = 0; b < blocks; ++b) {
+        starts[b] = k;
+        for (int i : lists[b]) it[k++] = items[i];
+    }
+    starts[blocks] = k;
+    out->table = tb;
+    out->table_bytes = bytes;
+    out->starts_off = starts_off;
+    out->items_off = items_off;
+    out->blocks = blocks;
+    out->n_jobs = n;
+    out->n_items = k;
+    out->max_list_kg = *std::max_element(kg.begin(), kg.end());
+    return hipSuccess;
+}
+
+static std::atomic<unsigned long long> g_many_launches{0};
+unsigned long long conv_wgrad_p16_many_launches() { return g_many_launches.load(); }
+
+hipError_t conv_wgrad_p16_many(const WgP16Many& m, const void* table_dev, hipStream_t st) {
+    if (m.table == nullptr || table_dev == nullptr || m.blocks < 1) return hipErrorInvalidValue;
+    ++g_many_launches;
+    const unsigned char* base = (const unsigned char*)table_dev;
+    hipLaunchKernelGGL(wgrad_p16_many_kernel<P16_WAVES>, dim3((unsigned)m.blocks), dim3(P16_WAVES * 64), 0, st,
+                       (const WgP16Desc*)base, (const int*)(base + m.starts_off),
+                       (const WgP16Item*)(base + m.items_off));
+    return hipGetLastError();
+}
+
+}
diff --git a/mandheling-dsp-training_amd/niti_amd/_lib.py b/mandheling-dsp-training_amd/niti_amd/_lib.py
--- a/mandheling-dsp-training_amd/niti_amd/_lib.py
+++ b/mandheling-dsp-training_amd/niti_amd/_lib.py
@@ -69,6 +69,11 @@
         "pad_r", "dilate_h", "dilate_w", "oh", "ow", "cip", "cop", "np")]
 
 
+class WgradP16Job(C.Structure):
+    _fields_ = [("g", Geom), ("x_p16", C.c_void_p), ("dy_p16", C.c_void_p), ("acc", C.c_void_p),
+                ("amax", C.c_void_p)]
+
+
 class EvalTotals(C.Structure):
     _fields_ = [("images", C.c_uint64), ("top1", C.c_uint64), ("topk", C.c_uint64), ("loss_sum", C.c_double)]
 
@@ -116,6 +121,8 @@
         "niti_diag_head_chain_launches": (C.c_ulonglong, []),
         "niti_diag_head_chain": (None, [C.c_int]),
         "niti_diag_p16_jobs_cap": (None, [C.c_int]),
+        "niti_diag_wgrad_batch": (None, [C.c_int]),
+        "niti_diag_wgrad_batch_launches": (C.c_ulonglong, []),
         "niti_tensor_convert": (ci, [tp, tp, vp]),
         "niti_geom_finalize": (ci, [C.POINTER(Geom)]),
         "niti_conv_workspace_bytes": (ci, [C.POINTER(Geom), ci, C.POINTER(C.c_size_t)]),
@@ -140,6 +147,8 @@
         "niti_diag_rowconv_stamps": (None, [vp]),
         "niti_conv_wgrad_p16_workspace": (ci, [C.POINTER(Geom), ci, C.POINTER(C.c_size_t)]),
         "niti_conv_wgrad_p16_acc": (ci, [C.POINTER(Geom), vp, vp, vp, vp, vp, C.c_size_t, ci, vp]),
+        "niti_conv_wgrad_p16_many_workspace": (ci, [C.POINTER(WgradP16Job), ci, ci, ci, C.POINTER(C.c_size_t)]),
+        "niti_conv_wgrad_p16_many": (ci, [C.POINTER(WgradP16Job), ci, ci, ci, vp, C.c_size_t, C.POINTER(ci), vp]),
         "niti_matmul_acc": (ci, [ci, ci, ci, vp, i64, vp, i64, vp, i64, vp, vp, C.c_size_t, vp]),
         "niti_absmax_i32": (ci, [vp, i64, vp, vp]),
         "niti_requant_act": (ci, [vp, i64, ci, vp, vp, vp, vp, ci, vp, vp, vp]),
diff --git a/mandheling-dsp-training_amd/niti_amd/ops.py b/mandheling-dsp-training_amd/niti_amd/ops.py
--- a/mandheling-dsp-training_amd/niti_amd/ops.py
+++ b/mandheling-dsp-training_amd/niti_amd/ops.py
@@ -349,6 +349,23 @@
     return acc
 
 
+def conv_wgrad_p16_many(jobs, blocks: int, t: int, stream=None):
+    n = len(jobs)
+    accs = [torch.zeros((g.c_out, g.kh, g.kw, g.cip), dtype=torch.int32, device=xP.device) for g, xP, _, _ in jobs]
+    arr = (L.WgradP16Job * n)()
+    for j, ((g, xP, dyP, amax), acc) in enumerate(zip(jobs, accs)):
+        arr[j].g = g
+        arr[j].x_p16, arr[j].dy_p16, arr[j].acc = xP.data_ptr(), dyP.data_ptr(), acc.data_ptr()
+        arr[j].amax = None if amax is None else amax.data_ptr()
+    nb = C.c_size_t()
+    check(L.lib().niti_conv_wgrad_p16_many_workspace(arr, n, blocks, t, C.byref(nb)), "p16 many workspace")
+    ws = torch.zeros(int(nb.value), dtype=torch.uint8, device=accs[0].device)
+    splits = (C.c_int * n)()
+    check(L.lib().niti_conv_wgrad_p16_many(arr, n, blocks, t, _ptr(ws), int(nb.value), splits, _stream(stream)),
+          "conv_wgrad_p16_many")
+    return accs, list(splits)
+
+
 def matmul_acc(B16, A16, ldc, amax=None, use_workspace=True, stream=None):
     m, k16 = B16.shape
     o = A16.shape[0]
```

Result: faster. 746,100 images/s, median of 6 (+8.0%).
